# jasperlinthorst/reveal

Hardware: AMD Instinct MI355X
Metric: Mbp/s indexed+MUM-anchored (reveal rem) (higher is better)
Workload: dtype int32

## Files before the change

include/reveal_amd.h:

```cpp
#ifndef REVEAL_AMD_H
#define REVEAL_AMD_H
#include <stdint.h>

#ifdef __cplusplus
extern "C" {
#endif

typedef struct rv_index rv_index;

const char *rv_last_error(void);
int  rv_abi_version(void);
int  rv_sa_bits(void);
int  rv_device_count(void);

rv_index *rv_new(int device);
void rv_free(rv_index *h);

int rv_add_sample(rv_index *h);
int rv_add_sequence(rv_index *h, const char *seq, int64_t len, int64_t *begin, int64_t *end);
int rv_reset(rv_index *h);
int rv_reserve_text(rv_index *h, int64_t bytes);
int64_t rv_n(const rv_index *h);
int rv_nsamples(const rv_index *h);
int rv_nnodes(const rv_index *h);
// ... 12 lines not shown
int64_t rv_getmultimums(rv_index *h, int minlength, int minn, int mems, int64_t *members);
int rv_fetch_multi(rv_index *h, uint32_t *l, int32_t *n, int64_t *off, uint16_t *so, int64_t *pos);

typedef struct {
    int64_t n;
    int32_t depth;
    int32_t nsamples;
    int32_t nnodes;
    int32_t parent;
    int32_t kind;
    int32_t reserved;
    int64_t nmums;
    int64_t nmembers;
} rv_sub;

int rv_align_begin(rv_index *h, int minl, int minn);
int rv_frontier_size(rv_index *h);
int rv_frontier_scan(rv_index *h);
int rv_sub_skip_scan(rv_index *h, int s);
int rv_sub_info(rv_index *h, int s, rv_sub *out);
int rv_sub_nodes(rv_index *h, int s, int64_t *begin_end );
int rv_sub_mums(rv_index *h, int s, uint32_t *l, int32_t *n, int64_t *off, uint16_t *so, int64_t *pos);
int64_t rv_sub_array(rv_index *h, int s, int which, void *out, int64_t cap);
int rv_sub_split(rv_index *h, int s, uint32_t l, int nsp, const int64_t *sp,
                 const int64_t *lead, int nlead, const int64_t *trail, int ntrail,
                 const int64_t *match, int nmatch, const int64_t *rest, int nrest);
int rv_frontier_commit(rv_index *h, int32_t *children);
int rv_align_end(rv_index *h);

typedef struct {
    int64_t steps;
    int64_t splits;
    int64_t anchored_bp;
    int32_t levels;
    int32_t maxdepth;
    int64_t scanned_ranks;
    double  t_scan, t_host, t_split, t_bubble;
} rv_align_stats;
int rv_align_builtin(rv_index *h, int minl, int minn, rv_align_stats *st);

int rv_align_builtin_until(rv_index *h, int minl, int minn, int stop_subs, rv_align_stats *st);
int rv_align_builtin_resume(rv_index *h, rv_align_stats *st);
int rv_align_builtin_continue(rv_index *h, int stop_subs, rv_align_stats *st);
int rv_frontier_counts(rv_index *h, int64_t *out);
int rv_frontier_export(rv_index *h, int64_t *meta, int64_t *node_first, int64_t *nodes);
int64_t rv_frontier_pack(rv_index *h, const int32_t *subs, int k, void *sa, void *lcp, void *bwt, int on_device);
int rv_frontier_import(rv_index *h, int minl, int minn, uint32_t maxlcp, int level, int nsubs, const int64_t *meta,
                       const int64_t *node_first, const int64_t *nodes, int64_t m,
                       const void *sa, const void *lcp, const void *bwt, int on_device);
int64_t rv_frontier_seeds_export(rv_index *h, const int32_t *subs, int k, int64_t *out, int64_t cap);
int rv_frontier_seeds_import(rv_index *h, int nsubs, const int64_t *words, int64_t nwords);
uint32_t rv_maxlcp(const rv_index *h);
int rv_cascade_info(const rv_index *h, int64_t *out);
const char *rv_cascade_why(const rv_index *h);
int64_t rv_anchor_count(rv_index *h, int64_t *members);
int rv_fetch_anchors(rv_index *h, uint32_t *l, int64_t *off, int64_t *pos);
int rv_set_result_buffers(rv_index *h, uint32_t *l, int64_t l_cap, int64_t *off, int64_t off_cap, int64_t *pos, int64_t pos_cap);
typedef struct {
    int64_t  key, n;
    int32_t  depth, nsamples, nnodes, picked;
    int64_t  nmums;
    uint32_t l; int32_t mn;
    int64_t  sp_min;
    uint64_t h_sa, h_lcp, h_mums;
} rv_trace;
int rv_set_trace(rv_index *h, int on);
int rv_set_preselect(rv_index *h, int64_t maxmums);
int rv_set_option(rv_index *h, const char *name, int64_t value);
int rv_get_option(rv_index *h, const char *name, int64_t *value);
int rv_set_launch_trace(int on);
int rv_option_count(void);
const char *rv_option_name(int k);
int64_t rv_trace_count(rv_index *h);
int rv_fetch_trace(rv_index *h, rv_trace *out, int64_t cap);

typedef struct rv_subindex rv_subindex;
rv_index *rv_clone(rv_index *h);
rv_subindex *rv_sx_main(rv_index *h);
rv_subindex *rv_sx_copy(rv_subindex *x);
void rv_sx_free(rv_subindex *x);
int rv_sx_info(const rv_subindex *x, rv_sub *out);
int rv_sx_nodes(const rv_subindex *x, int64_t *begin_end);
int64_t rv_sx_array(rv_subindex *x, int which, void *out, int64_t cap);
int64_t rv_sx_scan(rv_subindex *x, int minl, int minn, int64_t *members);
int rv_sx_fetch(rv_subindex *x, uint32_t *l, int32_t *n, int64_t *off, uint16_t *so, int64_t *pos);
int rv_sx_split(rv_subindex *x, const int64_t *lead, int nlead, const int64_t *trail, int ntrail,
                const int64_t *match, int nmatch, const int64_t *rest, int nrest, rv_subindex **out);
int rv_sx_extract(rv_subindex *x, int64_t *intervals, int niv);

int64_t rv_chain(int64_t m, int k, const uint32_t *len, const int32_t *nmem, const int64_t *crd, const int64_t *left,
                 const int64_t *right, int64_t wscore, int64_t wpen, int model, int64_t *out_idx, int64_t *out_score);

typedef struct { int64_t wscore, wpen, maxmums, seedsize; int gcmodel; int trim; double pcutoff; } rv_picker_args;
typedef struct {
    int picked; uint32_t pick_l; int32_t pick_n; int pick_members; uint16_t *pick_so; int64_t *pick_pos; int64_t member_cap;
    int64_t nleft, nright, nseed_members, seed_cap, seed_member_cap;
    uint32_t *seed_l; int32_t *seed_n; int64_t *seed_off; uint16_t *seed_so; int64_t *seed_pos; int64_t *seed_score; uint8_t *seed_right;
} rv_picker_out;
int rv_set_picker(rv_index *h, int kind, const rv_picker_args *args);
int rv_picker_info(const rv_index *h, int64_t *out);
int rv_pick_chain(const rv_picker_args *args, int nsub, int64_t m, const uint32_t *l, const int32_t *n, const int64_t *off, const uint16_t *so,
                  const int64_t *pos, int nsamples, const int64_t *seq_begin, const int64_t *iv_begin, const int64_t *iv_end, int minlength,
                  rv_picker_out *out);

typedef struct rv_graph rv_graph;
rv_graph *rv_graph_import(int64_t nnodes, const int64_t *node_b, const int64_t *node_e, const int8_t *node_aligned, const int8_t *node_sent,
// ... 83 lines not shown
```

reveal_amd/_index.py:

```python
import ctypes
import mmap
import os
import sys
import numpy as np

from . import _lib
from ._lib import RV_T, RV_SA, RV_SAI, RV_LCP, RV_SO, RV_NSEP


def _page_array(count, dtype):
    nbytes = max(int(count), 1) * np.dtype(dtype).itemsize
    m = mmap.mmap(-1, (nbytes + mmap.PAGESIZE - 1) // mmap.PAGESIZE * mmap.PAGESIZE)
    return np.frombuffer(m, dtype=dtype, count=max(int(count), 1))


def _pairs(iv, sa64):
    a = np.ascontiguousarray(np.array([(int(b), int(e)) for b, e in iv], dtype=np.int64).reshape(-1, 2))
    return a, len(a)


_OPTION_DEFAULTS = {}


def make_index_type(sa64, error):
# ... 523 lines not shown
        def picker_info(self):
            o = (ctypes.c_int64 * 6)()
            self._dll.rv_picker_info(self._h, o)
            return dict(kind=int(o[0]), calls=int(o[1]), seeded=int(o[2]), picker_s=o[3] / 1e9, lists_s=o[4] / 1e9, graphalign_s=o[5] / 1e9)

        def _result_buffers_free(self):
            c = self.__dict__.get("_res_bufs")
            if c is not None and sys.getrefcount(c[0]) == 2 and sys.getrefcount(c[1]) == 2 and sys.getrefcount(c[2]) == 2:
                return c
            return None

        def _offer_result_buffers(self):
            c = self._result_buffers_free()
            if c is not None:
                self._dll.rv_set_result_buffers(self._h, c[0].ctypes.data, len(c[0]), c[1].ctypes.data, len(c[1]), c[2].ctypes.data, len(c[2]))
            else:
                self._dll.rv_set_result_buffers(self._h, None, 0, None, 0, None, 0)

        def _builtin_result(self, st, trace):
            dll, h = self._dll, self._h
            mem = ctypes.c_int64(0)
            na = dll.rv_anchor_count(h, ctypes.byref(mem))
            c = self._result_buffers_free()
            if c is not None and len(c[0]) >= max(na, 1) and len(c[1]) >= na + 1 and len(c[2]) >= max(mem.value, 1):
                l, off, pos = c
            else:
                dll.rv_set_result_buffers(h, None, 0, None, 0, None, 0)
                if os.environ.get("RV_RESULT_BUFS", "") == "heap":
                    l = np.empty(max(na, 1), dtype=np.uint32); off = np.empty(na + 1, dtype=np.int64); pos = np.empty(max(mem.value, 1), dtype=np.int64)
                else:
                    l = _page_array(max(na, 1), np.uint32); off = _page_array(na + 1, np.int64); pos = _page_array(max(mem.value, 1), np.int64)
                self.__dict__["_res_bufs"] = (l, off, pos)
            c = None
            off[0] = 0
            if dll.rv_fetch_anchors(h, l.ctypes.data, off.ctypes.data, pos.ctypes.data) != 0:
                self._fail()
            tr = None
            if trace:
                nt = dll.rv_trace_count(h)
                tr = np.zeros(max(nt, 1), dtype=_lib.TRACE_DTYPE)
                if dll.rv_fetch_trace(h, tr.ctypes.data, len(tr)) != 0:
                    self._fail()
                tr = tr[:nt]
            stats = {f[0]: getattr(st, f[0]) for f in _lib.RvAlignStats._fields_}
            return dict(stats=stats, anchors=(l[:na], off[:na + 1], pos[:mem.value]), trace=tr)

        @property
        def maxlcp(self):
            return int(self._dll.rv_maxlcp(self._h))

        def cascade_info(self):
            o = np.zeros(8, dtype=np.int64)
            self._dll.rv_cascade_info(self._h, o.ctypes.data)
            return dict(done=bool(o[0]), levels=int(o[1]), matches=int(o[2]), witnesses=int(o[3]), subindices=int(o[4]), undecided=int(o[5]), rebuilt_ranks=int(o[6]), decided_from_witnesses=int(o[7]),
                        why=(self._dll.rv_cascade_why(self._h) or b"").decode())

        def align_builtin_until(self, stop_subs, minl=20, minn=2, trace=False):
            if not self._constructed:
                raise error("Index not yet constructed, alignment stopped.")
            self._dll.rv_set_trace(self._h, 1 if trace else 0)
            self._offer_result_buffers()
            self._st = _lib.RvAlignStats()
            self._trace = bool(trace)
            r = self._dll.rv_align_builtin_until(self._h, int(minl), int(minn), int(stop_subs), ctypes.byref(self._st))
            if r < 0:
                self._fail()
            self._pending = r > 0
            return r

        def align_builtin_continue(self, stop_subs):
            if not getattr(self, "_pending", False):
                return 0
            self._offer_result_buffers()
            r = self._dll.rv_align_builtin_continue(self._h, int(stop_subs), ctypes.byref(self._st))
            if r < 0:
                self._fail()
            self._pending = r > 0
            return r

        def frontier(self):
            c = np.zeros(4, dtype=np.int64)
            if self._dll.rv_frontier_counts(self._h, c.ctypes.data) != 0:
                self._fail()
            ns, m, nn, level = (int(x) for x in c)
            meta = np.zeros((max(ns, 1), 6), dtype=np.int64); nf = np.zeros(ns + 1, dtype=np.int64); nodes = np.zeros((max(nn, 1), 2), dtype=np.int64)
            if self._dll.rv_frontier_export(self._h, meta.ctypes.data, nf.ctypes.data, nodes.ctypes.data) != 0:
                self._fail()
            return dict(level=level, m=m, meta=meta[:ns], node_first=nf, nodes=nodes[:nn])

        def frontier_pack(self, subs, sa, lcp, bwt):
            subs = np.ascontiguousarray(subs, dtype=np.int32)
            ptr, dev = _pointers(sa, lcp, bwt)
            r = self._dll.rv_frontier_pack(self._h, subs.ctypes.data, len(subs), ptr[0], ptr[1], ptr[2], dev)
            if r < 0:
                self._fail()
            return int(r)

        def frontier_seeds(self, subs):
            subs = np.ascontiguousarray(subs, dtype=np.int32)
            need = self._dll.rv_frontier_seeds_export(self._h, subs.ctypes.data, len(subs), None, 0)
            if need < 0:
                self._fail()
            out = np.zeros(max(int(need), 1), dtype=np.int64)
            if self._dll.rv_frontier_seeds_export(self._h, subs.ctypes.data, len(subs), out.ctypes.data, int(need)) != need:
                self._fail()
            return out[:int(need)]

# ... 69 lines not shown
```

reveal_amd/_lib.py:

```python
import ctypes
import importlib.util
import os
import sys
import numpy as np

_HERE = os.path.dirname(os.path.abspath(__file__))

RV_T, RV_SA, RV_SAI, RV_LCP, RV_SO, RV_NSEP, RV_NODES = range(7)
K_SCAN_PAIR, K_SCAN_MULTI, K_SA_SORT, K_LCP, K_SPLIT, K_LABEL, K_BUBBLE, K_RADIX_SCATTER, K_RADIX_HIST, K_TEXT_ROUND, K_CASCADE, K_DIAG_TABLE, K_INIT_KEYS, K_PUBLISH = range(14)

c_i64p = ctypes.POINTER(ctypes.c_int64)
V = ctypes.c_void_p


class RvSub(ctypes.Structure):
    _fields_ = [("n", ctypes.c_int64), ("depth", ctypes.c_int32), ("nsamples", ctypes.c_int32),
                ("nnodes", ctypes.c_int32), ("parent", ctypes.c_int32), ("kind", ctypes.c_int32),
                ("reserved", ctypes.c_int32), ("nmums", ctypes.c_int64), ("nmembers", ctypes.c_int64)]


class RvAlignStats(ctypes.Structure):
    _fields_ = [("steps", ctypes.c_int64), ("splits", ctypes.c_int64), ("anchored_bp", ctypes.c_int64),
                ("levels", ctypes.c_int32), ("maxdepth", ctypes.c_int32), ("scanned_ranks", ctypes.c_int64),
                ("t_scan", ctypes.c_double), ("t_host", ctypes.c_double), ("t_split", ctypes.c_double),
# ... 3 lines not shown
TRACE_DTYPE = np.dtype([("key", np.int64), ("n", np.int64), ("depth", np.int32), ("nsamples", np.int32),
                        ("nnodes", np.int32), ("picked", np.int32), ("nmums", np.int64), ("l", np.uint32),
                        ("mn", np.int32), ("sp_min", np.int64), ("h_sa", np.uint64), ("h_lcp", np.uint64),
                        ("h_mums", np.uint64)], align=True)

_I, _L, _D = ctypes.c_int, ctypes.c_int64, ctypes.c_double
SYMBOLS = {
    "rv_last_error": (ctypes.c_char_p, []),
    "rv_abi_version": (_I, []),
    "rv_sa_bits": (_I, []),
    "rv_device_count": (_I, []),
    "rv_new": (V, [_I]),
    "rv_free": (None, [V]),
    "rv_add_sample": (_I, [V]),
    "rv_add_sequence": (_I, [V, ctypes.c_char_p, _L, c_i64p, c_i64p]),
    "rv_reset": (_I, [V]),
    "rv_reserve_text": (_I, [V, _L]),
    "rv_n": (_L, [V]),
    "rv_nsamples": (_I, [V]),
    "rv_nnodes": (_I, [V]),
    "rv_node_list": (_I, [V, V]),
    "rv_construct": (_I, [V, _I, ctypes.c_char_p, ctypes.c_char_p, _I]),
    "rv_upload": (_I, [V]),
    "rv_upload_again": (_I, [V]),
    "rv_get_array": (_L, [V, _I, V, _L]),
    "rv_getmums": (_L, [V, _I]),
    "rv_fetch_mums": (_I, [V, V, V, V, _L]),
    "rv_getmultimums": (_L, [V, _I, _I, _I, c_i64p]),
    "rv_fetch_multi": (_I, [V, V, V, V, V, V]),
    "rv_align_begin": (_I, [V, _I, _I]),
    "rv_frontier_size": (_I, [V]),
    "rv_frontier_scan": (_I, [V]),
    "rv_sub_skip_scan": (_I, [V, _I]),
    "rv_sub_info": (_I, [V, _I, ctypes.POINTER(RvSub)]),
    "rv_sub_nodes": (_I, [V, _I, V]),
    "rv_sub_mums": (_I, [V, _I, V, V, V, V, V]),
    "rv_sub_array": (_L, [V, _I, _I, V, _L]),
    "rv_sub_split": (_I, [V, _I, ctypes.c_uint32, _I, V, V, _I, V, _I, V, _I, V, _I]),
    "rv_frontier_commit": (_I, [V, V]),
    "rv_align_end": (_I, [V]),
    "rv_align_builtin": (_I, [V, _I, _I, ctypes.POINTER(RvAlignStats)]),
    "rv_align_builtin_until": (_I, [V, _I, _I, _I, ctypes.POINTER(RvAlignStats)]),
    "rv_align_builtin_resume": (_I, [V, ctypes.POINTER(RvAlignStats)]),
    "rv_align_builtin_continue": (_I, [V, _I, ctypes.POINTER(RvAlignStats)]),
    "rv_frontier_counts": (_I, [V, V]),
    "rv_frontier_export": (_I, [V, V, V, V]),
    "rv_frontier_pack": (_L, [V, V, _I, V, V, V, _I]),
    "rv_frontier_import": (_I, [V, _I, _I, ctypes.c_uint32, _I, _I, V, V, V, _L, V, V, V, _I]),
    "rv_frontier_seeds_export": (_L, [V, V, _I, V, _L]),
    "rv_frontier_seeds_import": (_I, [V, _I, V, _L]),
    "rv_maxlcp": (ctypes.c_uint32, [V]),
    "rv_cascade_info": (ctypes.c_int, [V, V]),
    "rv_cascade_why": (ctypes.c_char_p, [V]),
    "rv_anchor_count": (_L, [V, c_i64p]),
    "rv_fetch_anchors": (_I, [V, V, V, V]),
    "rv_set_result_buffers": (_I, [V, V, _L, V, _L, V, _L]),
    "rv_set_trace": (_I, [V, _I]),
    "rv_set_preselect": (_I, [V, _L]),
    "rv_set_option": (_I, [V, ctypes.c_char_p, _L]),
    "rv_set_launch_trace": (_I, [_I]),
    "rv_batch_new": (V, []),
    "rv_batch_add": (_I, [V, V]),
    "rv_batch_run": (_I, [V, _I, _I, _I, V, V]),
    "rv_batch_info": (_I, [V, V]),
    "rv_batch_free": (None, [V]),
    "rv_dev_alloc": (V, [_I, _L]),
    "rv_dev_free": (_I, [_I, V]),
    "rv_ipc_export": (_I, [_I, V, V]),
    "rv_ipc_open": (V, [_I, V]),
    "rv_ipc_close": (_I, [_I, V]),
    "rv_dev_copy": (_I, [_I, V, V, _L]),
    "rv_get_option": (_I, [V, ctypes.c_char_p, c_i64p]),
    "rv_option_count": (_I, []),
    "rv_option_name": (ctypes.c_char_p, [_I]),
    "rv_trace_count": (_L, [V]),
    "rv_fetch_trace": (_I, [V, V, _L]),
    "rv_clone": (V, [V]),
    "rv_sx_main": (V, [V]),
    "rv_sx_copy": (V, [V]),
    "rv_sx_free": (None, [V]),
    "rv_sx_info": (_I, [V, ctypes.POINTER(RvSub)]),
    "rv_sx_nodes": (_I, [V, V]),
    "rv_sx_array": (_L, [V, _I, V, _L]),
    "rv_sx_scan": (_L, [V, _I, _I, c_i64p]),
    "rv_sx_fetch": (_I, [V, V, V, V, V, V]),
    "rv_sx_split": (_I, [V, V, _I, V, _I, V, _I, V, _I, V]),
    "rv_sx_extract": (_I, [V, V, _I]),
    "rv_chain": (_L, [_L, _I, V, V, V, V, V, _L, _L, _I, V, V]),
    "rv_prof_enable": (_I, [V, _I]),
    "rv_prof_reset": (_I, [V]),
    "rv_prof_get": (_I, [V, _I, c_i64p, ctypes.POINTER(_D), ctypes.POINTER(_D)]),
    "rv_measure_bandwidth": (_I, [_I, _L, _I, ctypes.POINTER(_D), ctypes.POINTER(_D)]),
    "rv_sa_stats": (_I, [V] + [ctypes.POINTER(_I)] * 4 + [c_i64p, ctypes.POINTER(_I)]),
    "rv_sa_diag_table": (_I, [V]),
    "rv_sa_tail": (_I, [V, c_i64p]),
    "rv_set_picker": (_I, [V, _I, V]),
    "rv_picker_info": (_I, [V, c_i64p]),
    "rv_pick_chain": (_I, [V, _I, _L, V, V, V, V, V, _I, V, V, V, _I, V]),
    "rv_graph_import": (V, [_L, V, V, V, V, V, V, V, _L, V, V, V, V, V, V, _I, V, V, _I, V, _I]),
    "rv_graph_pick": (_I, [V, V, _I, _L, V, V, V, V, V, V, V, _I, V]),
    "rv_graph_align": (_I, [V, V, _L, V, V, ctypes.c_uint32, V, _I, V, V]),
    "rv_graph_align_fetch": (_I, [V, V]),
    "rv_graph_finish": (_I, [V]),
    "rv_set_graph_picker": (_I, [V, V, V]),
    "rv_graph_new": (V, []),
    "rv_graph_replay_begin": (V, [_I, V, V]),
# ... 104 lines not shown
```

reveal_amd/csrc/rv_align.hip:

```cpp
#include "rv_index.h"
#include "rv_split.h"
#include "rv_decide.h"
static_assert(RV_TSUB_TILE == RV_SPLIT_TILE, "one tile -> sub-index table serves the split passes and the multi-sample picker");
#include "rv_leaf.h"
#include "rv_cascade.h"
#include <string.h>
#include <algorithm>
#include <chrono>
#include <thread>
#include <atomic>
#include "rv_graphrem.h"

namespace {

double now_s() {
    return std::chrono::duration<double>(std::chrono::steady_clock::now().time_since_epoch()).count();
}

u64 hash_step(u64 acc, u64 i, int64_t v) {
    u64 x = (u64)v + (i + 1) * 0x9E3779B97F4A7C15ULL;
    x ^= x >> 30; x *= 0xbf58476d1ce4e5b9ULL;
    x ^= x >> 27; x *= 0x94d049bb133111ebULL;
    x ^= x >> 31;
    return acc + x;
// ... 114 lines not shown
    DBuf dD, dTab, dTile, dList, dFlag, dPar, dDbg, scrSA, scrLCP, scrBWT;
    RvCascadeBufs cas;
    RvCascadeOut cas_out{};
    DBuf dPbReady; u32 pb_epoch = 0;
    DBuf dNextTsub;
    DBuf dTmin;
    HBuf hLeafRoots[2], hLeafOut;
    DBuf dLeaf, dLeafRoots[2];
    hipStream_t leaf_stream = nullptr, leaf_stream2 = nullptr;
    hipStream_t bub_stream = nullptr, bub_stream2 = nullptr;
    hipEvent_t ev_fork = nullptr, ev_join = nullptr, ev_join2 = nullptr;
    hipEvent_t ev_ready = nullptr, ev_leaf[RV_LEVEL_BUFS + 1] = {}, ev_roots[2] = {nullptr, nullptr};
    bool roots_inflight[2] = {false, false};
    bool flag_clean = false;
    DBuf dDec, dErr, dTab0;
    bool next_dev_ok = false, cur_dev_ok = false, early_done = false, early_bubble = false, use_leaf = false;
    int64_t par_min_cur = RV_BUBBLE_PAR_N;
    const sa_t *d_next_nodes = nullptr; const uint8_t *d_next_flags = nullptr;
    std::vector<sa_t> next_nodes; std::vector<uint8_t> next_flags;
    bool leaf_pending[RV_LEVEL_BUFS + 1] = {};
    size_t leaf_anchor_cap = 0, leaf_trace_cap = 0;
    std::vector<uint8_t> leaf_done;
    std::vector<RvLeafRoot> leaf_roots[2];
    Packer pk;
    std::vector<int> stamp; int epoch = 0;
    std::vector<sa_t> cb, ce, mb, me, cut_lo, cut_hi, mend_pos;
    std::vector<uint8_t> cc;
    std::vector<int> ctab_first, mtab_first, cut_first, mend_first, split_subs;
    std::vector<u32> sub_off_h;
    std::vector<int> tile_sub;
    std::vector<int64_t> mpre, sub_start, woff, toff, next_ss;
    const int64_t *d_next_ss = nullptr;
    const int *d_next_want = nullptr;
    const int *d_next_tsub = nullptr;
    std::vector<int> next_tsub;
    std::vector<u32> pick_l; std::vector<sa_t> pick_pos;
    std::vector<u32> child_base, child_n;
    std::vector<RvBubbleDesc> descs;
    std::vector<std::vector<RvBubbleDesc>> rounds;
    std::vector<RvBubbleDesc> kids_small, kids_big, kids_lds;
    struct Kid { int64_t off, n; int c0, c1; int64_t m0, wsum; };
    std::vector<Kid> kid_tmp;
    std::vector<u32> an_l; std::vector<int64_t> an_off, an_pos;
    bool trace_on = false;
    std::vector<rv_trace> trace;
    rv_align_stats st{};
    double lg[8] = {0}, lgx[8] = {0}, lg_t0 = 0;
    int leaf_flip = 0;
    bool leaf_launch_due = false, hook_early = false;
    size_t last_leaf_count = 0;
    bool running = false;
    u32 *lf_counters = nullptr; unsigned long long *lf_stats = nullptr; u32 *lf_l = nullptr; int64_t *lf_pos = nullptr; rv_trace *lf_tr = nullptr;
    size_t early_sent = 0; u32 *early_l = nullptr; int64_t *early_pos = nullptr;
    size_t leaf_na = 0;
    void release() {
        if (leaf_stream) (void)hipStreamSynchronize(leaf_stream);
        if (leaf_stream2) (void)hipStreamSynchronize(leaf_stream2);
        if (bub_stream) { (void)hipStreamSynchronize(bub_stream); (void)hipStreamSynchronize(bub_stream2); }
        for (int k = 0; k < RV_LEVEL_BUFS; k++) { lvSA[k].release(); lvLCP[k].release(); lvBWT[k].release(); }
        scrSA.release(); scrLCP.release(); scrBWT.release(); cas.release();
        dTmin.release(); dPbReady.release(); dNextTsub.release(); dD.release(); dTab.release(); dTile.release(); dList.release(); dFlag.release(); dPar.release(); dDbg.release(); pk.release(); dDec.release(); dErr.release(); dTab0.release(); hLeafRoots[0].release(); hLeafRoots[1].release(); hLeafOut.release(); dLeaf.release(); dLeafRoots[0].release(); dLeafRoots[1].release();
        if (leaf_stream) { rv_stream_put(leaf_stream); leaf_stream = nullptr; }
        if (leaf_stream2) { rv_stream_put(leaf_stream2); leaf_stream2 = nullptr; }
        if (bub_stream) { rv_stream_put(bub_stream); bub_stream = nullptr; rv_stream_put(bub_stream2); bub_stream2 = nullptr; (void)hipEventDestroy(ev_fork); (void)hipEventDestroy(ev_join); (void)hipEventDestroy(ev_join2); ev_fork = ev_join = ev_join2 = nullptr; }
        if (ev_ready) { (void)hipEventDestroy(ev_ready); ev_ready = nullptr; }
        for (int k = 0; k <= RV_LEVEL_BUFS; k++) if (ev_leaf[k]) { (void)hipEventDestroy(ev_leaf[k]); ev_leaf[k] = nullptr; }
        for (int k = 0; k < 2; k++) if (ev_roots[k]) { (void)hipEventDestroy(ev_roots[k]); ev_roots[k] = nullptr; }
    }
};

void rv_align_free(rv_index *h) {
    if (h->al && h->al->feed) { (void)rv_replay_feed_finish(h->al->feed); h->al->feed = nullptr; }
    if (h->al) { h->al->release(); delete h->al; h->al = nullptr; }
}

static int report_dev_err(u32 err) {
    if (err & 1u) { rv_set_error("split: the intervals returned by graphalign do not partition the sub-index (child size mismatch)"); return -1; }
    if (err & 4u) { rv_set_error("device-side decision: a picked match does not lie inside the intervals of its sub-index"); return -1; }
    if (err & 2u) { rv_set_error("bubble_sort (data-parallel rounds): a mover found no landing site"); return -1; }
    if (err & 16u) { rv_set_error("bubble_sort (data-parallel rounds): a tile waited in vain for the tile above it (workgroups not dispatched in index order?)"); return -1; }
    if (err) { rv_set_error("device-side error word %u", err); return -1; }
    return 0;
}

static int64_t bubble_par_default(bool multi) { return multi ? (int64_t)262144 : (int64_t)RV_BUBBLE_PAR_N; }

static const sa_t *cur_sa(rv_index *h) { Align *a = h->al; return a->level == 0 ? h->dSA.as<sa_t>() : a->lvSA[a->cur].as<sa_t>(); }
static const lcp_t *cur_lcp(rv_index *h) { Align *a = h->al; return a->level == 0 ? h->dLCP.as<lcp_t>() : a->lvLCP[a->cur].as<lcp_t>(); }
static const uint8_t *cur_bwt(rv_index *h) { Align *a = h->al; return a->level == 0 ? h->dBWT.as<uint8_t>() : a->lvBWT[a->cur].as<uint8_t>(); }

static int sample_of(const rv_index *h, int64_t pos) {
    return (int)(std::lower_bound(h->nsep.begin(), h->nsep.end(), pos) - h->nsep.begin());
}

static int count_samples(rv_index *h, const RvIntv *iv, size_t cnt) {
    Align *a = h->al;
    if (h->nsamples > 2) {
        bool sorted = true;
        for (size_t k = 1; k < cnt && sorted; k++) sorted = iv[k - 1].begin <= iv[k].begin;
        if (sorted) {
            int ns = 0, last = -1; size_t sp = 0;
            for (size_t k = 0; k < cnt; k++) {
                while (sp < h->nsep.size() && h->nsep[sp] < iv[k].begin) sp++;
                if ((int)sp != last) { ns++; last = (int)sp; }
            }
            return ns;
// ... 1119 lines not shown
    if (!a->multi && cm.m_next > 1) {
        a->d_err = a->dErr.as<u32>();
    } else {
        u32 err = 0;
        RV_HIP(hipMemcpyAsync(&err, a->dErr.p, 4, hipMemcpyDeviceToHost, q));
        RV_HIP(hipStreamSynchronize(q));
        RV_TRY(report_dev_err(err));
    }

    if (a->level == 0) h->main_arrays_freed = true;
    a->level++;
    a->cur = cm.nxt;
    a->cur_dev_ok = a->next_dev_ok; a->early_done = false; a->early_bubble = false;
    std::swap(a->lv, a->nx);
    a->dec.reset(a->lv.size());
    a->skip_scan.assign((size_t)a->lv.size(), 0);
    a->st.t_split += t1 - t0;
    a->st.t_bubble += now_s() - t1;
    return 0;
}

static int builtin_leaf_setup(rv_index *h) {
    Align *a = h->al;
    hipStream_t q = h->ws.stream;
    a->use_leaf = !a->multi && !h->ws.opt.no_leaf && a->picker == 0;
    a->leaf_flip = 0;
    if (!a->use_leaf) return 0;
    a->leaf_anchor_cap = (size_t)(h->nT / std::max(a->minl, 1)) + 1024;
    a->leaf_trace_cap = a->trace_on ? 2 * a->leaf_anchor_cap + 1024 : 0;
    const size_t bytes = 256 + a->leaf_anchor_cap * (4 + 8 + 8) + a->leaf_trace_cap * sizeof(rv_trace) + 64;
    RV_TRY(a->dLeaf.reserve(bytes));
    uint8_t *base = a->dLeaf.as<uint8_t>();
    a->lf_counters = (u32 *)base;
    a->lf_stats = (unsigned long long *)(base + 64);
    a->lf_pos = (int64_t *)(base + 256); a->lf_l = (u32 *)(a->lf_pos + 2 * a->leaf_anchor_cap);
    a->lf_tr = (rv_trace *)(base + 256 + a->leaf_anchor_cap * 20 + ((8 - (a->leaf_anchor_cap * 20) % 8) % 8));
    RV_HIP(hipMemsetAsync(base, 0, 256, q));
    if (!a->leaf_stream) {
        RV_HIP(rv_stream_get(&a->leaf_stream));
        RV_HIP(rv_stream_get(&a->leaf_stream2));
        RV_HIP(hipEventCreateWithFlags(&a->ev_ready, hipEventDisableTiming));
        for (int k = 0; k <= RV_LEVEL_BUFS; k++) RV_HIP(hipEventCreateWithFlags(&a->ev_leaf[k], hipEventDisableTiming));
        for (int k = 0; k < 2; k++) RV_HIP(hipEventCreateWithFlags(&a->ev_roots[k], hipEventDisableTiming));
    }
    for (int k = 0; k <= RV_LEVEL_BUFS; k++) a->leaf_pending[k] = false;
    a->roots_inflight[0] = a->roots_inflight[1] = false;
    return 0;
}

static int builtin_setup(rv_index *h, int minl, int minn) {
    RV_TRY(align_begin(h, minl, minn, h->al && h->al->trace_on));
    Align *a = h->al;
    a->full_only = !a->trace_on && a->picker == 0;
    a->an_l.clear(); a->an_off.assign(1, 0); a->an_pos.clear(); a->trace.clear(); a->leaf_na = 0; a->early_sent = 0;
    a->seeds_cur.clear(); a->seeds_lead.clear(); a->seeds_trail.clear(); a->picker_calls = a->picker_seeded = 0; a->picker_ns = a->picker_list_ns = a->galign_ns = 0;
    if (a->picker == 1) {
        if ((int)h->nodes.size() != h->nsamples) { rv_set_error("the native picker (rv_set_picker) takes one sequence per sample: %d sequences in %d samples", (int)h->nodes.size(), h->nsamples); return -1; }
        if (h->rc) { rv_set_error("the native picker (rv_set_picker) with construct(rc=1) is not supported"); return -1; }
    }
    if (a->picker != 0 && a->multi && !a->trace_on) { a->presel_on = true; a->pick_filter = true; }
    else a->pick_filter = false;
    if (a->picker == 2) {
        if (!a->ggraph) { rv_set_error("rv_set_graph_picker: no graph"); return -1; }
        if (h->rc) { rv_set_error("the native picker (rv_set_graph_picker) with construct(rc=1) is not supported"); return -1; }
        a->g_left.assign((size_t)a->lv.size(), RvGraphIv{-1, -1}); a->g_right.assign((size_t)a->lv.size(), RvGraphIv{-1, -1});
    }
    const bool use_leaf = !a->multi && !h->ws.opt.no_leaf && a->picker == 0;
    a->use_leaf = use_leaf;
    if (!a->multi && a->full_only && h->n < ((int64_t)1 << 32)) {
        prep_level_tables(h, a->lv, h->n);
        if (a->next_dev_ok) {
            a->pk.clear();
            RV_TRY(publish_next_tables(h, a->dTab0, a->lv.nsamples, false));
            a->cur_dev_ok = true;
        }
    }
    RV_TRY(builtin_leaf_setup(h));
    a->running = true;
    return 0;
}

struct PickScratch {
    std::vector<u32> pk_l, pk_sl; std::vector<int32_t> pk_n, pk_sn; std::vector<int64_t> pk_off, pk_mpos, pk_sb, pk_ib, pk_ie, pk_soff, pk_spos, pk_ssc;
    std::vector<uint16_t> pk_mso, pk_sso; std::vector<uint8_t> pk_srt;
};
struct PickRes {
    int rc = -9;
    u32 l = 0; int members = 0;
    std::vector<uint16_t> so; std::vector<int64_t> pos;
    double t_list = 0, t_pick = 0;
    std::string err;
};
static void pick_one(rv_index *h, int s, PickScratch &X, PickRes &R, RvGraphIv gleft = RvGraphIv{-1, -1}, RvGraphIv gright = RvGraphIv{-1, -1}) {
    Align *a = h->al;
    const Level &lv = a->lv;
    const int W = h->nsamples, want = lv.nsamples[(size_t)s];
    const RvIntv *nodes = lv.nodes.data() + lv.node_first[(size_t)s];
    const size_t nn = (size_t)(lv.node_first[(size_t)s + 1] - lv.node_first[(size_t)s]);
    const int64_t first = a->mum_first[(size_t)s], cnt = a->nmums[(size_t)s];
    Align::SeedList &sl = a->seeds_lead[(size_t)s], &st = a->seeds_trail[(size_t)s];
    R.so.assign((size_t)W, 0); R.pos.assign((size_t)W, 0);
    const double tp0 = now_s();
    X.pk_l.clear(); X.pk_n.clear(); X.pk_off.assign(1, 0); X.pk_mso.clear(); X.pk_mpos.clear();
    if (!a->multi) {
        for (int64_t k = first; k < first + cnt; k++) {
            const RvPairRec &r = a->recs[(size_t)k];
            X.pk_l.push_back(r.l); X.pk_n.push_back(2);
// ... 312 lines not shown
            fprintf(stderr, "level %3d subs %7d (leaf %7zu) ranks %10lld | leafprep %6.1f scan %6.1f host %6.1f | commit: tables %6.1f upload %6.1f split-enq %6.1f bubble-enq %6.1f | drain %7.1f us | next biggest %lld\n",
                    log_level, log_ns, log_leaf, (long long)log_m, (tl_leaf - tl0) * 1e6, (t0 - tl_leaf) * 1e6, (tl1 - t0) * 1e6,
                    a->lg[0] * 1e6, (a->lg[1] - a->lg[0]) * 1e6, (a->lg[2] - a->lg[1]) * 1e6, (tl2 - tl1) * 1e6 - a->lg[2] * 1e6, (tl3 - tl2) * 1e6,
                    (long long)biggest);
        }
    }
    RV_HIP(hipStreamSynchronize(q));
    if (a->lv.size() > 0) {
        u32 err = 0;
        RV_HIP(hipMemcpy(&err, a->dErr.p, 4, hipMemcpyDeviceToHost));
        if (err & 1u) { rv_set_error("split: the intervals returned by graphalign do not partition the sub-index (child size mismatch)"); return -1; }
        if (err) { rv_set_error("device-side error %u in the level before the hand-off", err); return -1; }
    }
    return 0;
}

static void fill_offsets(int64_t *off, size_t na, int64_t base) {
    const int nt = na > ((size_t)1 << 18) ? 4 : 1;
    std::vector<std::thread> th;
    for (int t = 1; t < nt; t++) {
        const size_t lo = na / nt * t, hi = t + 1 == nt ? na : na / nt * (t + 1);
        th.emplace_back([=]() { for (size_t k = lo; k < hi; k++) off[k] = base + 2 * (int64_t)(k + 1); });
    }
    for (size_t k = 0; k < na / nt; k++) off[k] = base + 2 * (int64_t)(k + 1);
    for (auto &x : th) x.join();
}
static int builtin_finish(rv_index *h, rv_align_stats *out) {
    Align *a = h->al;
    hipStream_t q = h->ws.stream;
    h->rb.direct = false;
    if (a->use_leaf && a->running) {
        u32 *lf_counters = a->lf_counters; u32 *lf_l = a->lf_l; int64_t *lf_pos = a->lf_pos; rv_trace *lf_tr = a->lf_tr;
        RV_HIP(hipStreamSynchronize(a->leaf_stream));
        RV_HIP(hipStreamSynchronize(a->leaf_stream2));
        for (int k = 0; k <= RV_LEVEL_BUFS; k++) a->leaf_pending[k] = false;
        RV_TRY(a->hLeafOut.reserve(256));
        RV_HIP(hipMemcpyAsync(a->hLeafOut.p, lf_counters, 128, hipMemcpyDeviceToHost, q));
        RV_HIP(hipStreamSynchronize(q));
        u32 cnt[4]; unsigned long long stv[8];
        memcpy(cnt, a->hLeafOut.p, sizeof cnt); memcpy(stv, a->hLeafOut.as<uint8_t>() + 64, sizeof stv);
        if (h->ws.opt.leaf_prof)
            fprintf(stderr, "leaf: steps %llu splits %llu | cycles idle %llu scan %llu split %llu bubble %llu\n", stv[0], stv[1], stv[4], stv[5], stv[6], stv[7]);
        if (cnt[2]) { rv_set_error(cnt[2] & 4u ? "leaf kernel: recursion stack overflow" : "leaf kernel: a sub-index does not match its intervals"); return -1; }
        if (cnt[0] > a->leaf_anchor_cap || cnt[1] > a->leaf_trace_cap) { rv_set_error("leaf kernel: output buffer too small"); return -1; }
        a->leaf_na = 0;
        if (cnt[0]) {
            const size_t na = cnt[0];
            const size_t nl = a->an_l.size(), np = a->an_pos.size();
            rv_index::ResultBufs &rb = h->rb;
            rb.direct = rb.l && (int64_t)(nl + na) <= rb.l_cap && (int64_t)(nl + na + 1) <= rb.off_cap && (int64_t)(np + 2 * na) <= rb.pos_cap;
            int64_t *pp; u32 *pl;
            if (rb.direct) { pp = rb.pos + np; pl = rb.l + nl; }
            else { RV_TRY(a->hLeafOut.reserve(na * 20 + 64)); pp = a->hLeafOut.as<int64_t>(); pl = (u32 *)(pp + 2 * na); }
            const size_t sent = (rb.direct && a->early_l == pl && a->early_pos == pp) ? std::min(a->early_sent, na) : 0;
            if (sent < na) {
                RV_HIP(hipMemcpyAsync(pp + 2 * sent, lf_pos + 2 * sent, (na - sent) * 16, hipMemcpyDeviceToHost, a->leaf_stream));
                RV_HIP(hipMemcpyAsync(pl + sent, lf_l + sent, (na - sent) * 4, hipMemcpyDeviceToHost, a->leaf_stream));
            }
            RV_TRY(rv_ensure_working_text(h));
            RV_TRY(rv_leaf_lower_launch(h->ws, h->dT.as<uint8_t>(), lf_pos, lf_l, (u32)na));
            if (rb.direct) fill_offsets(rb.off + nl + 1, na, (int64_t)np);
            RV_HIP(hipStreamSynchronize(a->leaf_stream));
            RV_HIP(hipStreamSynchronize(q));
            a->leaf_na = na;
        }
        if (a->trace_on && cnt[1]) {
            const size_t at = a->trace.size();
            a->trace.resize(at + cnt[1]);
            RV_HIP(hipMemcpy(a->trace.data() + at, lf_tr, (size_t)cnt[1] * sizeof(rv_trace), hipMemcpyDeviceToHost));
        }
        a->st.steps += (int64_t)stv[0]; a->st.splits += (int64_t)stv[1]; a->st.anchored_bp += (int64_t)stv[2];
        if ((int64_t)stv[3] > a->st.maxdepth) a->st.maxdepth = (int32_t)stv[3];
    }
    a->running = false;
    if (out) *out = a->st;
    return 0;
}

static int install_frontier(rv_index *h, int level, int nsubs, const int64_t *meta, const int64_t *node_first, const int64_t *nodes, int64_t m,
                            const void *sa, const void *lcp, const void *bwt, int on_device);
static int builtin_cascade(rv_index *h) {
    Align *a = h->al;
    memset(&a->cas_out, 0, sizeof a->cas_out);
    if (a->trace_on || h->rc != 0 || h->n <= RV_LEAF_N || a->minl < 4 || h->ws.opt.no_cascade || a->picker != 0) return 0;
    const bool second_try = !a->multi && a->use_leaf && h->ws.opt.cascade_second == 2;
    auto interval_cascade = [&]() -> int {
        RvCascadeMultiOut mo;
        RV_TRY(rv_cascade_multi_run(h, a->cas, a->minl, &mo));
        a->cas_out.done = mo.done; a->cas_out.levels = mo.levels; a->cas_out.cands = mo.cands; a->cas_out.witnesses = mo.witnesses; a->cas_out.children = mo.children;
        a->cas_out.undecided = mo.undecided; a->cas_out.rebuilt_ranks = mo.rebuilt_ranks; a->cas_out.why = mo.why;
        if (!mo.done) return 0;
        const int k = h->nsamples;
        a->st.splits += (int64_t)mo.an_l.size(); a->st.steps += mo.steps; a->st.levels += mo.levels; a->st.scanned_ranks += h->n;
        if (mo.maxdepth > a->st.maxdepth) a->st.maxdepth = mo.maxdepth;
        h->main_arrays_freed = true;
        if (mo.undecided > 0) {
            RV_TRY(install_frontier(h, 1, (int)mo.undecided, mo.meta.data(), mo.node_first.data(), mo.nodes.data(), mo.rebuilt_ranks, mo.d_sa, mo.d_lcp, mo.d_bwt, 1));
        } else {
            a->lv.clear();
            a->level = 1;
        }
        {
            const size_t na = mo.an_l.size(), l0 = a->an_l.size(), p0 = a->an_pos.size(), o0 = a->an_off.size();
            a->an_l.insert(a->an_l.end(), mo.an_l.begin(), mo.an_l.end());
            a->an_pos.resize(p0 + na * (size_t)k);
            for (size_t x = 0; x < na * (size_t)k; x++) a->an_pos[p0 + x] = (int64_t)mo.an_pos[x];
            a->an_off.resize(o0 + na);
            for (size_t x = 0; x < na; x++) a->an_off[o0 + x] = (int64_t)(p0 + (x + 1) * (size_t)k);
            int64_t bp = 0;
            for (size_t x = 0; x < na; x++) bp += mo.an_l[x];
            a->st.anchored_bp += bp;
            (void)l0;
        }
        return 0;
    };
    if (a->multi || second_try) return interval_cascade();
    if (!a->use_leaf) return 0;
    RvCascadeIO io;
    io.anchor_count = a->lf_counters; io.anchor_cap = (u32)a->leaf_anchor_cap; io.anchor_l = a->lf_l; io.anchor_pos = a->lf_pos;
    io.stats = a->lf_stats; io.leaf_err = a->lf_counters + 2;
    io.stage_cap = (u32)h->ws.opt.leaf_acap;
    RvCascadeHost hx;
    hx.side = a->leaf_stream;
    a->early_sent = 0;
    if (h->rb.l) {
        const int64_t nl = (int64_t)a->an_l.size(), np = (int64_t)a->an_pos.size();
        const int64_t room = std::min(std::min(h->rb.l_cap - nl, h->rb.off_cap - nl - 1), (h->rb.pos_cap - np) / 2);
        if (room > 0) { hx.l = h->rb.l + nl; hx.pos = h->rb.pos + np; hx.cap = (u32)std::min<int64_t>(room, 0xffffffffll); }
    }
    io.lvSA = &a->lvSA[0]; io.lvLCP = &a->lvLCP[0]; io.lvBWT = &a->lvBWT[0]; io.roots = &a->dLeafRoots[0];
    const int dmode = (int)h->ws.opt.cascade_danger;
    RV_TRY(rv_cascade_run(h, a->cas, io, a->minl, &a->cas_out, dmode == 2 ? 1 : 0, 0, &hx));
    if (!a->cas_out.done && a->cas_out.undecided > 0 && dmode == 1) {
        RV_HIP(hipMemsetAsync(a->dLeaf.p, 0, 256, h->ws.stream));
        RV_TRY(rv_cascade_run(h, a->cas, io, a->minl, &a->cas_out, 1, 1, &hx));
    }
    if (!a->cas_out.done) {
        if (hx.l) RV_HIP(hipStreamSynchronize(a->leaf_stream));
        RV_HIP(hipMemsetAsync(a->dLeaf.p, 0, 256, h->ws.stream));
        if (a->cas_out.undecided > 0 && !h->ws.opt.cascade_second_off) return interval_cascade();
        return 0;
    }
    a->st.levels += a->cas_out.levels;
    a->st.scanned_ranks += h->n;
    a->early_sent = a->cas_out.sent; a->early_l = hx.l; a->early_pos = hx.pos;
    if (!a->cas.lin_rest.empty() && h->nodes.size() > 2) {
        std::vector<RvIntv> rest, gone;
        for (size_t k = 0; k + 1 < a->cas.lin_rest.size(); k += 2) rest.push_back({a->cas.lin_rest[k], a->cas.lin_rest[k + 1]});
        std::sort(rest.begin(), rest.end(), intv_less);
        for (const RvIntv &v : h->nodes) {
            if (v.end <= v.begin) continue;
            const auto it = std::lower_bound(rest.begin(), rest.end(), v, intv_less);
            if (it == rest.end() || it->begin != v.begin) gone.push_back(v);
        }
        RV_TRY(add_decision(h, 0, 0, nullptr, 0, gone.data(), (int)gone.size(), nullptr, 0, nullptr, 0, rest.data(), (int)rest.size()));
        a->dec.drop_lead = true;
        RV_TRY(rv_frontier_commit(h, nullptr));
        for (size_t s2 = 0; s2 < a->lv.depth.size(); s2++) a->lv.depth[s2] = a->cas.lin_rest_depth;
        return 0;
    }
    h->main_arrays_freed = true;
    a->level = 1;
    a->lv.clear();
    return 0;
}

int rv_cascade_info(const rv_index *h, int64_t *out) {
    for (int k = 0; k < 8; k++) out[k] = 0;
    if (!h->al) return 0;
    const RvCascadeOut &c = h->al->cas_out;
    out[0] = c.done ? 1 : 0; out[1] = c.levels; out[2] = c.cands; out[3] = c.witnesses; out[4] = c.children; out[5] = c.undecided; out[6] = c.rebuilt_ranks; out[7] = c.solved;
    return 0;
}

const char *rv_cascade_why(const rv_index *h) {
    if (!h->al || h->al->cas_out.done || !h->al->cas_out.why) return "";
    return h->al->cas_out.why;
}

int rv_align_builtin(rv_index *h, int minl, int minn, rv_align_stats *out) {
    RV_TRY(builtin_setup(h, minl, minn));
    Align *a = h->al;
    if (a->replay_graph && a->picker == 1) {
        a->feed = rv_replay_feed_start(a->replay_graph);
        a->fed = 0;
        a->replay_graph = nullptr;
        if (!a->feed) return -1;
    }
    int rc = builtin_cascade(h);
    if (rc == 0) rc = builtin_levels(h, 0);
    if (rc == 0) rc = builtin_finish(h, out);
    if (a->feed) {
        RvReplayFeed *f = a->feed; a->feed = nullptr;
        if (rc == 0) { if (rv_replay_feed_finish(f) != 0) return -1; }
        else { const std::string keep = rv_last_error(); (void)rv_replay_feed_finish(f); rv_set_error("%s", keep.c_str()); }
    }
    return rc;
}

int rv_align_builtin_until(rv_index *h, int minl, int minn, int stop_subs, rv_align_stats *out) {
    RV_TRY(builtin_setup(h, minl, minn));
    RV_TRY(builtin_cascade(h));
    RV_TRY(builtin_levels(h, stop_subs));
    Align *a = h->al;
    if (a->lv.size() == 0) { RV_TRY(builtin_finish(h, out)); return 0; }
    if (out) *out = a->st;
    return a->lv.size();
}

int rv_align_builtin_continue(rv_index *h, int stop_subs, rv_align_stats *out) {
    RV_TRY(need_align(h));
    if (!h->al->running) { rv_set_error("no built-in run in progress (rv_align_builtin_until / rv_frontier_import)"); return -1; }
    if (stop_subs < 1) { rv_set_error("rv_align_builtin_continue: stop_subs must be positive"); return -1; }
    RV_HIP(hipSetDevice(h->device));
    Align *a = h->al;
    RV_TRY(builtin_levels(h, std::max(stop_subs, a->lv.size() + 1)));
    if (a->lv.size() == 0) { RV_TRY(builtin_finish(h, out)); return 0; }
    if (out) *out = a->st;
    return a->lv.size();
}

int rv_align_builtin_resume(rv_index *h, rv_align_stats *out) {
    RV_TRY(need_align(h));
    if (!h->al->running) { rv_set_error("no built-in run in progress (rv_align_builtin_until / rv_frontier_import)"); return -1; }
// ... 77 lines not shown
    a->level = std::max(level, 1);
    a->cur = 0;
    RV_TRY(a->lvSA[0].reserve((size_t)(m + 64) * sizeof(sa_t)));
    RV_TRY(a->lvLCP[0].reserve((size_t)(m + 64) * sizeof(lcp_t)));
    RV_TRY(a->lvBWT[0].reserve((size_t)m + 64));
    const hipMemcpyKind kind = on_device ? hipMemcpyDeviceToDevice : hipMemcpyHostToDevice;
    if (m) {
        RV_HIP(hipMemcpyAsync(a->lvSA[0].p, sa, (size_t)m * sizeof(sa_t), kind, q));
        RV_HIP(hipMemcpyAsync(a->lvLCP[0].p, lcp, (size_t)m * sizeof(lcp_t), kind, q));
        RV_HIP(hipMemcpyAsync(a->lvBWT[0].p, bwt, (size_t)m, kind, q));
    }
    prep_level_tables(h, lv, m);
    a->pk.clear();
    RV_TRY(publish_next_tables(h, a->dTab0, lv.nsamples, false));
    RV_HIP(hipStreamSynchronize(q));
    a->cur_dev_ok = a->next_dev_ok; a->early_done = false; a->early_bubble = false;
    a->scanned = false; a->d_err = nullptr;
    a->dec.reset(lv.size());
    a->skip_scan.assign((size_t)lv.size(), 0);
    a->seeds_cur.clear(); a->seeds_lead.clear(); a->seeds_trail.clear();
    return 0;
}


int rv_frontier_import(rv_index *h, int minl, int minn, uint32_t maxlcp, int level, int nsubs, const int64_t *meta,
                       const int64_t *node_first, const int64_t *nodes, int64_t m, const void *sa, const void *lcp, const void *bwt, int on_device) {
    RV_HIP(hipSetDevice(h->device));
    if (h->nsamples < 2) { rv_set_error("align needs at least two samples"); return -1; }
    if (nsubs < 0 || m < 0 || m >= ((int64_t)1 << 32)) { rv_set_error("rv_frontier_import: bad sizes"); return -1; }
    const bool fresh = !(h->al && h->al->running);
    if (fresh) {
        if (h->text_only) h->maxlcp = maxlcp;
        else if (!h->constructed || h->main_arrays_freed) RV_TRY(rv_text_only(h, maxlcp));
        const bool keep_trace = h->al && h->al->trace_on;
        if (!h->al) h->al = new Align();
        Align *a = h->al;
        a->trace_on = keep_trace;
        a->minl = minl; a->minn = minn;
        a->multi = h->nsamples > 2;
        a->scanned = false; a->d_err = nullptr; a->flag_clean = false;
        a->next_dev_ok = a->cur_dev_ok = a->early_done = a->early_bubble = false;
        a->par_min_cur = (h->ws.opt.bubble_par_min >= 0 ? h->ws.opt.bubble_par_min : bubble_par_default(a->multi));
        RV_TRY(a->dErr.reserve(64));
        memset(&a->st, 0, sizeof a->st);
        a->full_only = !a->trace_on && a->picker == 0;
        a->pick_filter = a->picker != 0 && a->multi && !a->trace_on;
        if (a->pick_filter) a->presel_on = true;
        if (a->picker == 2) { rv_set_error("rv_frontier_import: a run on a graph (rv_set_graph_picker) is not handed off -- its sub-indices share the graph"); return -1; }
        if (a->picker == 1) {
            if ((int)h->nodes.size() != h->nsamples) { rv_set_error("the native picker (rv_set_picker) takes one sequence per sample: %d sequences in %d samples", (int)h->nodes.size(), h->nsamples); return -1; }
            if (h->rc) { rv_set_error("the native picker (rv_set_picker) with construct(rc=1) is not supported"); return -1; }
        }
        a->picker_calls = a->picker_seeded = 0; a->picker_ns = a->picker_list_ns = a->galign_ns = 0;
        a->an_l.clear(); a->an_off.assign(1, 0); a->an_pos.clear(); a->trace.clear(); a->leaf_na = 0; a->early_sent = 0;
        RV_TRY(builtin_leaf_setup(h));
    }
    RV_TRY(install_frontier(h, level, nsubs, meta, node_first, nodes, m, sa, lcp, bwt, on_device));
    h->al->running = true;
    return 0;
}

int64_t rv_frontier_seeds_export(rv_index *h, const int32_t *subs, int k, int64_t *out, int64_t cap) {
    if (need_align(h)) return -1;
    const Align *a = h->al;
    const int ns = a->lv.size();
    int64_t need = 0;
    for (int pass = 0; pass < 2; pass++) {
        int64_t at = 0;
        for (int i = 0; i < k; i++) {
            const int s = subs[i];
            if (s < 0 || s >= ns) { rv_set_error("sub-index %d out of range", s); return -1; }
            const Align::SeedList *sd = (s < (int)a->seeds_cur.size() && a->seeds_cur[(size_t)s].size() > 0) ? &a->seeds_cur[(size_t)s] : nullptr;
            if (pass) out[at] = sd ? (int64_t)sd->size() : 0;
            at++;
            if (!sd) continue;
            for (size_t r = 0; r < sd->size(); r++) {
                const int64_t mem = sd->off[r + 1] - sd->off[r];
                if (pass) {
                    out[at] = sd->l[r]; out[at + 1] = sd->n[r]; out[at + 2] = sd->score[r]; out[at + 3] = mem;
                    for (int64_t q2 = 0; q2 < mem; q2++) { out[at + 4 + 2 * q2] = sd->so[(size_t)(sd->off[r] + q2)]; out[at + 5 + 2 * q2] = sd->pos[(size_t)(sd->off[r] + q2)]; }
                }
                at += 4 + 2 * mem;
            }
        }
        need = at;
        if (!out || cap < need) break;
    }
    return need;
}

int rv_frontier_seeds_import(rv_index *h, int nsubs, const int64_t *words, int64_t nwords) {
    RV_TRY(need_align(h));
    Align *a = h->al;
    if (!a->running || nsubs != a->lv.size()) { rv_set_error("rv_frontier_seeds_import: %d seed lists for a frontier of %d sub-indices", nsubs, a->lv.size()); return -1; }
    if (a->picker != 1) { rv_set_error("rv_frontier_seeds_import: seeds belong to the native picker (rv_set_picker)"); return -1; }
    std::vector<Align::SeedList> nxt((size_t)nsubs);
    int64_t at = 0;
    for (int s = 0; s < nsubs; s++) {
        if (at >= nwords) { rv_set_error("rv_frontier_seeds_import: truncated seed lists"); return -1; }
        const int64_t cnt = words[at++];
        if (cnt < 0) { rv_set_error("rv_frontier_seeds_import: bad seed count"); return -1; }
        for (int64_t r = 0; r < cnt; r++) {
            if (at + 4 > nwords) { rv_set_error("rv_frontier_seeds_import: truncated seed lists"); return -1; }
            const int64_t l = words[at], n = words[at + 1], sc = words[at + 2], mem = words[at + 3];
            if (mem < 0 || mem > h->nsamples || at + 4 + 2 * mem > nwords) { rv_set_error("rv_frontier_seeds_import: bad seed record"); return -1; }
            std::vector<uint16_t> so((size_t)mem); std::vector<int64_t> pos((size_t)mem);
            for (int64_t q2 = 0; q2 < mem; q2++) {
// ... 350 lines not shown
```

reveal_amd/csrc/rv_cascade.h:

```cpp
#pragma once
#include "rv_common.h"
#include <vector>

struct RvCascadeBufs {
    DBuf d[40];
    HBuf hstage, hstage2;
    u32 M = 0, NW = 0;
    u32 lin_roots = 0, lin_picks = 0, lin_nA = 0, lin_nB = 0;
    int64_t lin_steps = 0; int lin_maxdepth = 0; size_t lin_off[6] = {0, 0, 0, 0, 0, 0};
    std::vector<int64_t> lin_rest; int lin_rest_depth = 0;
    hipStream_t prio_stream = nullptr; hipEvent_t ev_in = nullptr, ev_out = nullptr;
    void release() {
        for (auto &b : d) b.release(); hstage.release(); hstage2.release();
        if (prio_stream) { (void)hipStreamDestroy(prio_stream); prio_stream = nullptr; }
        if (ev_in) { (void)hipEventDestroy(ev_in); ev_in = nullptr; }
        if (ev_out) { (void)hipEventDestroy(ev_out); ev_out = nullptr; }
    }
};

struct RvCascadeIO {
    u32 *anchor_count; u32 anchor_cap; u32 *anchor_l; int64_t *anchor_pos;
    unsigned long long *stats;
    u32 *leaf_err;
    u32 stage_cap;
    DBuf *lvSA, *lvLCP, *lvBWT, *roots;
};

struct RvCascadeHost {
    hipStream_t side = nullptr;
    int64_t *pos = nullptr; u32 *l = nullptr; u32 cap = 0;
};

struct RvCascadeOut {
    bool done;
    int levels;
    int64_t cands, witnesses, children, undecided, rebuilt_ranks;
    int64_t solved, unsolved;
    const char *why;
    u32 sent;
};

#define RV_CASM_K 16
struct RvCascadeMultiOut {
    bool done; int levels; int64_t cands, witnesses, children, undecided, rebuilt_ranks, steps; int maxdepth; const char *why;
    int64_t big, big_ranks;
    std::vector<u32> an_l; std::vector<int64_t> an_pos;
    std::vector<int64_t> meta, node_first, nodes;
    const void *d_sa, *d_lcp, *d_bwt;
};

struct rv_index;
struct RvBatchGroup;
RvBatchGroup *rv_batch_group_new(int device);
void rv_batch_group_begin(RvBatchGroup *g, int total);
void rv_batch_group_leave(RvBatchGroup *g);
void rv_batch_group_free(RvBatchGroup *g);
void rv_batch_group_info(const RvBatchGroup *g, int64_t *out);
int rv_cascade_multi_run(rv_index *h, RvCascadeBufs &cb, int minl, RvCascadeMultiOut *out);
int rv_cascade_run(rv_index *h, RvCascadeBufs &cb, const RvCascadeIO &io, int minl, RvCascadeOut *out, int danger = 0, int reuse = 0,
                   const RvCascadeHost *host = nullptr);
```

reveal_amd/csrc/rv_cascade.hip:

```cpp
#include "rv_index.h"
#include "rv_cascade.h"
#include "rv_leaf.h"
#include <algorithm>
#include <string.h>
#include <stdio.h>
#include <stdlib.h>
#include <chrono>

namespace {

constexpr int TB = 256;
constexpr u32 NONE = 0xFFFFFFFFu;
#ifdef RV_SA64
constexpr int KEY_SHIFT = 40;
#else
constexpr int KEY_SHIFT = 32;
#endif
constexpr u64 KEY_LOW = (1ull << KEY_SHIFT) - 1;

struct CasIv { sa_t a0, a1, b0, b1; };
struct CasRes { sa_t qa, qb; u32 ql, lead, trail, state; };
enum { C_NCHILD = 0, C_NUND = 1, C_NWIT = 2, C_ERR = 3, C_MAXN = 4, C_LO = 5, C_HI = 6, C_LEVELS = 7, C_NSOLVED = 8, C_NUNSOLVED = 9, C_NRETRY = 10, C_TICKET = 11,
       C_NANCH = 12  };

__device__ inline bool cas_cut(const CasIv &iv, int64_t pa, int64_t pb, int64_t len, int64_t minl, int64_t *qa, int64_t *qb, int64_t *ql) {
    const int64_t ka = (int64_t)iv.a0 - pa, kb = (int64_t)iv.b0 - pb;
    int64_t k = ka > kb ? ka : kb;
    k = k > 0 ? k : 0;
    const int64_t a = pa + k, b = pb + k;
    int64_t l = len - k;
    const int64_t ra = (int64_t)iv.a1 - a, rb = (int64_t)iv.b1 - b;
    l = l < ra ? l : ra;
    l = l < rb ? l : rb;
    *qa = a; *qb = b; *ql = l;
    return l >= minl;
}
__device__ inline u64 cas_key(int64_t qa, int64_t ql) { return ((u64)ql << KEY_SHIFT) | (KEY_LOW - (u64)qa); }

__device__ inline u64 shfl_up64(u64 v, int d) {
    const u32 lo = __shfl_up((u32)v, d, 64), hi = __shfl_up((u32)(v >> 32), d, 64);
    return ((u64)hi << 32) | lo;
}
__device__ inline void seg_atomic_max64(u64 *__restrict__ dst, u32 child, u64 val, bool active) {
    const int lane = threadIdx.x & 63;
    if (!active) { child = NONE; val = 0; }
    val = rv_wave_seg_max_u64(child, val);
    const u32 nc = __shfl_down(child, 1, 64);
    const bool last = lane == 63 || nc != child;
    if (active && last && val > dst[child]) atomicMax((unsigned long long *)&dst[child], (unsigned long long)val);
}
__device__ inline void seg_atomic_max32(u32 *__restrict__ dst, u32 child, u32 val, bool active) {
    const int lane = threadIdx.x & 63;
    if (!active) { child = NONE; val = 0; }
    val = rv_wave_seg_max_u32(child, val);
    const u32 nc = __shfl_down(child, 1, 64);
    const bool last = lane == 63 || nc != child;
    if (active && last && val > dst[child]) atomicMax(&dst[child], val);
}

constexpr int WT_ITEMS = 8;
constexpr int WT_TILE = TB * WT_ITEMS;
constexpr int WT_REGIONS = 64;
__global__ __launch_bounds__(TB) void k_cas_witness(const sa_t *__restrict__ SA, const lcp_t *__restrict__ LCP, const uint8_t *__restrict__ BWT, int64_t n,
                                                    u32 minl, sa_t *__restrict__ w_pos, u32 *__restrict__ w_val, u32 *__restrict__ w_rank, u32 cap , u32 *__restrict__ counters ) {
    __shared__ __attribute__((aligned(16))) u32 sl0[WT_TILE + 8];
    __shared__ __attribute__((aligned(16))) uint8_t ss0[WT_TILE + 32];
    u32 *const sl = sl0 + 3;
    uint8_t *const ss = ss0 + 15;
    const int64_t j0 = (int64_t)blockIdx.x * WT_TILE;
    if (j0 + WT_TILE + 2 <= n && sizeof(lcp_t) == 4) {
        const uint4 *L4 = reinterpret_cast<const uint4 *>(LCP + j0);
        uint4 *d4 = reinterpret_cast<uint4 *>(sl + 1);
        for (int k = threadIdx.x; k < WT_TILE / 4; k += TB) d4[k] = L4[k];
        const uint4 *B4 = reinterpret_cast<const uint4 *>(BWT + j0);
        for (int k = threadIdx.x; k < WT_TILE / 16; k += TB) {
            uint4 v = B4[k];
            v.x = (v.x >> 7) & 0x01010101u; v.y = (v.y >> 7) & 0x01010101u; v.z = (v.z >> 7) & 0x01010101u; v.w = (v.w >> 7) & 0x01010101u;
            reinterpret_cast<uint4 *>(ss + 1)[k] = v;
        }
        if (threadIdx.x == 0) { sl[0] = j0 > 0 ? (u32)LCP[j0 - 1] : 0u; ss[0] = j0 > 0 ? (uint8_t)(BWT[j0 - 1] >> 7) : (uint8_t)0; }
        if (threadIdx.x == 1) { sl[WT_TILE + 1] = (u32)LCP[j0 + WT_TILE]; ss[WT_TILE + 1] = (uint8_t)(BWT[j0 + WT_TILE] >> 7); }
        if (threadIdx.x == 2) sl[WT_TILE + 2] = (u32)LCP[j0 + WT_TILE + 1];
    } else {
        for (int k = threadIdx.x; k < WT_TILE + 3; k += TB) { const int64_t j = j0 - 1 + k; sl[k] = (j >= 0 && j < n) ? (u32)LCP[j] : 0u; }
        for (int k = threadIdx.x; k < WT_TILE + 2; k += TB) { const int64_t j = j0 - 1 + k; ss[k] = (j >= 0 && j < n) ? (uint8_t)(BWT[j] >> 7) : (uint8_t)0; }
    }
    __syncthreads();
    const int lane = threadIdx.x & 63;
    const u64 lt = (lane == 0) ? 0ull : (~0ull >> (64 - lane));
#pragma unroll 1
    for (int r = 0; r < WT_ITEMS; r++) {
        const int k = r * TB + threadIdx.x;
        const int64_t j = j0 + k;
        const u32 lm1 = sl[k], l0 = sl[k + 1], l1 = sl[k + 2], l2 = sl[k + 3];
        const u32 sm1 = ss[k], s0 = ss[k + 1], s1 = ss[k + 2];
        const bool pair0 = (j >= 1) & (l0 > lm1) & (l0 > l1) & (s0 != sm1);
        const bool pair1 = (j + 1 < n) & (l1 > l0) & (l1 > l2) & (s1 != s0);
        const u32 w = pair0 ? (lm1 > l1 ? lm1 : l1) : pair1 ? (l0 > l2 ? l0 : l2) : (l0 > l1 ? l0 : l1);
        const bool hit = (j < n) & (w >= minl);
        const u64 bal = __ballot(hit);
        if (bal) {
            const u32 reg = blockIdx.x & (WT_REGIONS - 1);
            u32 base = 0;
            if (lane == 0) base = atomicAdd(&counters[reg], (u32)__popcll(bal));
            base = (u32)__shfl((int)base, 0, 64);
            if (hit) {
                const u32 i = base + (u32)__popcll(bal & lt);
                if (i < cap) { w_pos[(size_t)reg * cap + i] = SA[j]; w_val[(size_t)reg * cap + i] = w; w_rank[(size_t)reg * cap + i] = (u32)j; }
            }
        }
    }
}
__global__ __launch_bounds__(TB) void k_cas_wpack(const sa_t *__restrict__ src_pos, const u32 *__restrict__ src_val, const u32 *__restrict__ src_rank, u32 rcap,
                                                  const u32 *__restrict__ region_cnt, const u32 *__restrict__ region_off, sa_t *__restrict__ w_pos, u32 *__restrict__ w_val,
                                                  u32 *__restrict__ w_rank) {
    const u32 reg = blockIdx.y, i = blockIdx.x * TB + threadIdx.x;
    if (i >= region_cnt[reg]) return;
    const size_t f = (size_t)reg * rcap + i;
    const u32 o = region_off[reg] + i;
    w_pos[o] = src_pos[f]; w_val[o] = src_val[f]; w_rank[o] = src_rank[f];
}
__global__ __launch_bounds__(TB) void k_cas_wkeys(const u32 *__restrict__ w_rank, u32 NW, u64 *__restrict__ keys, u32 *__restrict__ vals) {
    const u32 i = blockIdx.x * TB + threadIdx.x;
    if (i < NW) { keys[i] = (u64)w_rank[i]; vals[i] = i; }
}
__global__ __launch_bounds__(TB) void k_cas_wgather(const sa_t *__restrict__ src_pos, const u32 *__restrict__ src_val, const u32 *__restrict__ perm, u32 NW,
                                                    sa_t *__restrict__ w_pos, u32 *__restrict__ w_val) {
    const u32 i = blockIdx.x * TB + threadIdx.x;
    if (i < NW) { const u32 f = perm[i]; w_pos[i] = src_pos[f]; w_val[i] = src_val[f]; }
}

__global__ __launch_bounds__(TB) void k_cas_keys(const RvPairRec *__restrict__ recs, u32 M, u64 *__restrict__ keys, u32 *__restrict__ vals) {
    const u32 i = blockIdx.x * TB + threadIdx.x;
    if (i < M) { keys[i] = (u64)recs[i].a; vals[i] = i; }
}
__global__ __launch_bounds__(TB) void k_cas_gather(const RvPairRec *__restrict__ recs, const u32 *__restrict__ perm, u32 M, sa_t *__restrict__ c_pa,
                                                   sa_t *__restrict__ c_pb, u32 *__restrict__ c_len, u32 *__restrict__ c_child) {
    const u32 i = blockIdx.x * TB + threadIdx.x;
    if (i >= M) return;
    const RvPairRec r = recs[perm[i]];
    c_pa[i] = r.a; c_pb[i] = r.b; c_len[i] = r.l; c_child[i] = 0u;
}
__global__ void k_cas_init(CasIv *__restrict__ iv, u64 *__restrict__ best, u32 *__restrict__ wmax, int32_t *__restrict__ depth, CasRes *__restrict__ res,
                           u32 *__restrict__ counters, CasIv root, u32 *__restrict__ w_child, u32 nw, u64 *__restrict__ dbest, u32 *__restrict__ dflag, u64 *__restrict__ dceil) {
    const u32 i = blockIdx.x * blockDim.x + threadIdx.x;
    if (i == 0) {
        if (dbest) { dbest[0] = 0; dflag[0] = 0; dceil[0] = 0; }
        iv[0] = root; best[0] = 0; wmax[0] = 0; depth[0] = 0;
        CasRes r; r.qa = 0; r.qb = 0; r.ql = 0; r.lead = NONE; r.trail = NONE; r.state = 0;
        res[0] = r;
        counters[C_NCHILD] = 1; counters[C_NUND] = 0; counters[C_ERR] = 0; counters[C_MAXN] = 0; counters[C_LO] = 0; counters[C_HI] = 1; counters[C_LEVELS] = 0; counters[C_NSOLVED] = 0; counters[C_NUNSOLVED] = 0; counters[C_NRETRY] = 0; counters[C_TICKET] = 0;
    }
    if (i < nw) w_child[i] = 0u;
}

struct CasRootTabs { const sa_t *beginA, *beginB; const int32_t *pickA, *pickB; const u32 *rootLead, *rootTrail; u32 nA, nB; };
__device__ inline int cas_contig_of(const sa_t *__restrict__ begins, u32 cnt, int64_t pos) {
    u32 lo = 0, hi = cnt;
    while (lo < hi) { const u32 mid = (lo + hi) >> 1; if ((int64_t)begins[mid] <= pos) lo = mid + 1; else hi = mid; }
    return (int)lo - 1;
}
__global__ void k_cas_init_roots(CasIv *__restrict__ iv, u64 *__restrict__ best, u32 *__restrict__ wmax, int32_t *__restrict__ depth, CasRes *__restrict__ res,
                                 u32 *__restrict__ counters, const CasIv *__restrict__ roots, const int32_t *__restrict__ rdepth, u32 nroots,
                                 u64 *__restrict__ dbest, u32 *__restrict__ dflag, u64 *__restrict__ dceil) {
    const u32 i = blockIdx.x * blockDim.x + threadIdx.x;
    if (i == 0) {
        counters[C_NCHILD] = nroots; counters[C_NUND] = 0; counters[C_ERR] = 0; counters[C_MAXN] = 0; counters[C_LO] = 0; counters[C_HI] = nroots; counters[C_LEVELS] = 0;
        counters[C_NSOLVED] = 0; counters[C_NUNSOLVED] = 0; counters[C_NRETRY] = 0; counters[C_TICKET] = 0;
    }
    if (i < nroots) {
        if (dbest) { dbest[i] = 0; dflag[i] = 0; dceil[i] = 0; }
        iv[i] = roots[i]; best[i] = 0; wmax[i] = 0; depth[i] = rdepth[i];
// ... 2 lines not shown
    }
}
__global__ __launch_bounds__(TB) void k_cas_assign_roots(const sa_t *__restrict__ c_pa, const sa_t *__restrict__ c_pb, const u32 *__restrict__ c_len, u32 *__restrict__ c_child, u32 M,
                                                         const sa_t *__restrict__ w_pos, u32 *__restrict__ w_child, u32 NW, const CasIv *__restrict__ roots, CasRootTabs t, int64_t minl) {
    const u32 i = blockIdx.x * TB + threadIdx.x;
    if (i < M) {
        const int64_t pa = (int64_t)c_pa[i], pb = (int64_t)c_pb[i], len = (int64_t)c_len[i];
        const int ca = cas_contig_of(t.beginA, t.nA, pa), cb = cas_contig_of(t.beginB, t.nB, pb);
        u32 c = NONE;
        if (ca >= 0 && cb >= 0 && t.pickA[ca] >= 0 && t.pickA[ca] == t.pickB[cb]) {
            const u32 k = (u32)t.pickA[ca];
            int64_t qa, qb, ql;
            if (t.rootLead[k] != NONE && cas_cut(roots[t.rootLead[k]], pa, pb, len, minl, &qa, &qb, &ql)) c = t.rootLead[k];
            else if (t.rootTrail[k] != NONE && cas_cut(roots[t.rootTrail[k]], pa, pb, len, minl, &qa, &qb, &ql)) c = t.rootTrail[k];
        }
        c_child[i] = c;
    }
    if (i < NW) {
        const int64_t pos = (int64_t)w_pos[i];
        const bool a_side = t.nB == 0 || pos < (int64_t)t.beginB[0];
        const int ct = a_side ? cas_contig_of(t.beginA, t.nA, pos) : cas_contig_of(t.beginB, t.nB, pos);
        u32 c = NONE;
        if (ct >= 0) {
            const int32_t k = a_side ? t.pickA[ct] : t.pickB[ct];
            if (k >= 0) {
                for (int which = 0; which < 2 && c == NONE; which++) {
                    const u32 r = which ? t.rootTrail[k] : t.rootLead[k];
                    if (r == NONE) continue;
                    const CasIv p = roots[r];
                    if ((pos >= (int64_t)p.a0 && pos < (int64_t)p.a1) || (pos >= (int64_t)p.b0 && pos < (int64_t)p.b1)) c = r;
                }
            }
        }
        w_child[i] = c;
    }
}
__global__ void k_cas_lineage_stats(unsigned long long *__restrict__ stats, unsigned long long steps, unsigned long long maxdepth) {
    if (threadIdx.x == 0 && blockIdx.x == 0) { atomicAdd(&stats[0], steps); atomicMax(&stats[3], maxdepth); }
}
__global__ __launch_bounds__(TB) void k_cas_lkeys(const sa_t *__restrict__ c_pa, const u32 *__restrict__ c_len, u32 M, u64 *__restrict__ keys, u32 *__restrict__ vals) {
    const u32 i = blockIdx.x * TB + threadIdx.x;
    if (i < M) { keys[i] = (((1ull << (64 - KEY_SHIFT)) - 1ull - (u64)c_len[i]) << KEY_SHIFT) | (u64)c_pa[i]; vals[i] = i; }
}
__global__ __launch_bounds__(TB) void k_cas_lgather(const sa_t *__restrict__ c_pa, const sa_t *__restrict__ c_pb, const u32 *__restrict__ c_len, const u32 *__restrict__ perm, u32 M,
                                                    sa_t *__restrict__ o_pa, sa_t *__restrict__ o_pb, u32 *__restrict__ o_len) {
    const u32 i = blockIdx.x * TB + threadIdx.x;
    if (i < M) { const u32 f = perm[i]; o_pa[i] = c_pa[f]; o_pb[i] = c_pb[f]; o_len[i] = c_len[f]; }
}

constexpr int CAS_ITEMS = 4;
__global__ __launch_bounds__(TB) void k_cas_assign(const sa_t *__restrict__ c_pa, const sa_t *__restrict__ c_pb, const u32 *__restrict__ c_len, u32 *__restrict__ c_child,
                                                   u32 M, const sa_t *__restrict__ w_pos, const u32 *__restrict__ w_val, u32 *__restrict__ w_child, u32 NW,
                                                   const CasIv *__restrict__ iv, const CasRes *__restrict__ res, u64 *__restrict__ best, u32 *__restrict__ wmax,
                                                   int64_t minl, int first, const u64 *__restrict__ ceil ) {
    const u32 mblocks = (M + TB * CAS_ITEMS - 1) / (TB * CAS_ITEMS);
    for (int it = 0; it < CAS_ITEMS; it++) {
    if (blockIdx.x < mblocks) {
        const u32 i = (blockIdx.x * CAS_ITEMS + (u32)it) * TB + threadIdx.x;
        u32 c = i < M ? c_child[i] : NONE;
        bool live = c != NONE;
        u64 key = 0;
        if (live) {
            const int64_t pa = (int64_t)c_pa[i], pb = (int64_t)c_pb[i], len = (int64_t)c_len[i];
            int64_t qa, qb, ql;
            if (!first) {
                const CasRes r = res[c];
                const CasIv p = iv[c];
                u32 nc = NONE;
                if (r.state == 1u) {
                    CasIv lv; lv.a0 = p.a0; lv.a1 = r.qa; lv.b0 = p.b0; lv.b1 = r.qb;
                    CasIv tv; tv.a0 = (sa_t)((int64_t)r.qa + r.ql); tv.a1 = p.a1; tv.b0 = (sa_t)((int64_t)r.qb + r.ql); tv.b1 = p.b1;
                    if (r.lead != NONE && cas_cut(lv, pa, pb, len, minl, &qa, &qb, &ql)) nc = r.lead;
                    else if (r.trail != NONE && cas_cut(tv, pa, pb, len, minl, &qa, &qb, &ql)) nc = r.trail;
                } else if (r.state == 3u) {
                    if (cas_cut(p, pa, pb, len, minl, &qa, &qb, &ql)) nc = r.lead;
                }
                c = nc;
                c_child[i] = c;
                live = c != NONE;
            } else {
                live = cas_cut(iv[c], pa, pb, len, minl, &qa, &qb, &ql);
                if (!live) { c = NONE; c_child[i] = NONE; }
            }
            if (live) key = cas_key(qa, ql);
        }
        bool bid = live;
        if (live && ceil) { const u64 ce = ceil[c]; bid = ce == 0 || key < ce; }
        seg_atomic_max64(best, c, key, bid);
    } else {
        const u32 i = ((blockIdx.x - mblocks) * CAS_ITEMS + (u32)it) * TB + threadIdx.x;
        u32 c = i < NW ? w_child[i] : NONE;
        bool live = c != NONE;
        u32 v = 0;
        if (live) {
            const int64_t pos = (int64_t)w_pos[i];
            v = w_val[i];
            if (!first) {
                const CasRes r = res[c];
                const CasIv p = iv[c];
                u32 nc = NONE;
                if (r.state == 1u) {
                    const int64_t ea = (int64_t)r.qa + r.ql, eb = (int64_t)r.qb + r.ql;
                    const bool in_lead = (pos >= p.a0 && pos < r.qa) || (pos >= p.b0 && pos < r.qb);
                    const bool in_trail = (pos >= ea && pos < p.a1) || (pos >= eb && pos < p.b1);
                    nc = in_lead ? r.lead : in_trail ? r.trail : NONE;
                } else if (r.state == 3u) nc = r.lead;
                c = nc;
                w_child[i] = c;
                live = c != NONE;
            } else {
                const CasIv p = iv[c];
                live = (pos >= p.a0 && pos < p.a1) || (pos >= p.b0 && pos < p.b1);
                if (!live) { c = NONE; w_child[i] = NONE; }
            }
        }
        seg_atomic_max32(wmax, c, v, live);
    }
    }
}

__global__ __launch_bounds__(TB) void k_cas_winner(const sa_t *__restrict__ c_pa, const sa_t *__restrict__ c_pb, const u32 *__restrict__ c_len,
                                                   const u32 *__restrict__ c_child, u32 M, const CasIv *__restrict__ iv, CasRes *__restrict__ res,
                                                   const u64 *__restrict__ best, int64_t minl) {
    const u32 i = blockIdx.x * TB + threadIdx.x;
    if (i >= M) return;
    const u32 c = c_child[i];
    if (c == NONE) return;
    int64_t qa, qb, ql;
    if (!cas_cut(iv[c], (int64_t)c_pa[i], (int64_t)c_pb[i], (int64_t)c_len[i], minl, &qa, &qb, &ql)) return;
    if (cas_key(qa, ql) == best[c]) { res[c].qa = (sa_t)qa; res[c].qb = (sa_t)qb; res[c].ql = (u32)ql; }
}

constexpr u32 DWALK = 1024;
struct CasDanger { u64 *best; u32 *flag; sa_t *qb; u64 *ceil; u32 *m1, *p1, *m2; u64 *key; const uint8_t *T0; const lcp_t *LCP; const u64 *rank; u32 leaf_n; uint8_t *dflag; const uint8_t *wcls; };
__device__ inline bool cas_is_danger(const CasIv &p, u64 bk, u32 wm, u32 minl, u32 leaf_n, u32 *theta) {
    const int64_t la = (int64_t)p.a1 - p.a0, lb = (int64_t)p.b1 - p.b0;
    const u32 bl = (u32)(bk >> KEY_SHIFT);
    const bool can = (la >= (int64_t)minl) & (lb >= (int64_t)minl);
    const bool split = can & (bl >= minl) & (bl > wm);
    *theta = bl >= minl ? bl : minl;
    return can & !split & (wm >= minl) & ((u64)(la + lb) > (u64)leaf_n);
}
__global__ __launch_bounds__(TB) void k_cas_dmark(const CasIv *__restrict__ iv, const u64 *__restrict__ best, const u32 *__restrict__ wmax, u32 minl, const u32 *__restrict__ counters, CasDanger dg) {
    const u32 lo = counters[C_LO], hi = counters[C_HI];
    for (u32 id = lo + blockIdx.x * TB + threadIdx.x; id < hi; id += gridDim.x * TB) {
        u32 theta;
        dg.dflag[id] = cas_is_danger(iv[id], best[id], wmax[id], minl, dg.leaf_n, &theta) ? 1 : 0;
    }
}
__global__ __launch_bounds__(TB) void k_cas_dwalk(const sa_t *__restrict__ w_pos, const u32 *__restrict__ w_val, const u32 *__restrict__ w_child, u32 NW,
                                                  const CasIv *__restrict__ iv, const u64 *__restrict__ best, const u32 *__restrict__ wmax, u32 minl, CasDanger dg) {
    const u32 i = blockIdx.x * TB + threadIdx.x;
    if (i >= NW) return;
    if (dg.wcls && dg.wcls[i]) return;
    const u32 c = w_child[i];
    if (c == NONE || !dg.dflag[c]) return;
    dg.m1[i] = 0; dg.key[i] = 0;
    const CasIv p = iv[c];
    u32 theta;
    if (!cas_is_danger(p, best[c], wmax[c], minl, dg.leaf_n, &theta)) return;
    const int64_t pos = (int64_t)w_pos[i];
    const int64_t cap = (pos < (int64_t)p.a1 ? (int64_t)p.a1 : (int64_t)p.b1) - pos;
    if (w_val[i] < theta || cap < (int64_t)theta) return;
    u32 b1 = 0, b2 = 0, part = NONE;
    bool over = false;
#pragma unroll 1
    for (int dir = -1; dir <= 1; dir += 2) {
        u32 steps = 0;
        u64 rk = dg.rank[i];
        u32 run = 0xFFFFFFFFu;
        for (int64_t k = (int64_t)i + dir; k >= 0 && k < (int64_t)NW; k += dir) {
            const u64 r2 = dg.rank[k];
            if (r2 != rk + (u64)(int64_t)dir) break;
            const u32 g = (u32)dg.LCP[dir > 0 ? r2 : rk];
            run = g < run ? g : run;
            rk = r2;
            if (run < theta) break;
            if (++steps > DWALK) { over = true; break; }
// ... 85 lines not shown
                u32 l = (u32)(cap < ck ? cap : ck);
                l = run < l ? run : l;
                if (l > b1) { b2 = b1; b1 = l; part = s0 + (u32)k; }
                else if (l > b2) b2 = l;
                if (run <= b2) break;
            }
        }
        dg.m1[i] = b1 >= theta ? b1 : 0u; dg.p1[i] = part; dg.m2[i] = b2;
    }
}
__global__ __launch_bounds__(TB) void k_cas_dpick(const sa_t *__restrict__ w_pos, const u32 *__restrict__ w_val, const u32 *__restrict__ w_child, u32 NW,
                                                  const CasIv *__restrict__ iv, const CasRes *__restrict__ res, const u64 *__restrict__ best, const u32 *__restrict__ wmax,
                                                  u32 minl, CasDanger dg) {
    const u32 i = blockIdx.x * TB + threadIdx.x;
    if (i >= NW) return;
    const u32 c = w_child[i];
    if (c == NONE || !dg.dflag[c]) return;
    const CasIv p = iv[c];
    u32 theta;
    const u64 bk = best[c];
    if (!cas_is_danger(p, bk, wmax[c], minl, dg.leaf_n, &theta)) return;
    const int64_t pos = (int64_t)w_pos[i];
    const int64_t cap = (pos < (int64_t)p.a1 ? (int64_t)p.a1 : (int64_t)p.b1) - pos;
    if (w_val[i] < theta || cap < (int64_t)theta) return;
    if ((u32)(bk >> KEY_SHIFT) >= minl) { const CasRes r = res[c]; if (pos == (int64_t)r.qa || pos == (int64_t)r.qb) atomicOr(&dg.flag[c], 1u); }
    const u32 b1 = dg.m1[i];
    if (b1 == 0) return;
    const u32 w = dg.p1[i];
    if (dg.m1[w] != b1 || dg.p1[w] != i || b1 <= dg.m2[i] || b1 <= dg.m2[w]) return;
    const int64_t pw = (int64_t)w_pos[w];
    const bool a_side = pos < (int64_t)p.a1, w_a_side = pw < (int64_t)p.a1;
    if (!a_side || w_a_side) return;
    const int64_t qa = pos, qb = pw;
    if (!(qa == (int64_t)p.a0 || qb == (int64_t)p.b0)) {
        const uint8_t ca = dg.T0[qa - 1];
        if (ca == dg.T0[qb - 1] && ca != 'N' && ca != '$' && !(ca >= 'a' && ca <= 'z')) return;
    }
    const u64 key = cas_key(qa, (int64_t)b1);
    dg.key[i] = key;
    if (key > dg.best[c]) atomicMax((unsigned long long *)&dg.best[c], (unsigned long long)key);
}
__global__ __launch_bounds__(TB) void k_cas_dwrite(const sa_t *__restrict__ w_pos, const u32 *__restrict__ w_child, u32 NW, CasDanger dg) {
    const u32 i = blockIdx.x * TB + threadIdx.x;
    if (i >= NW) return;
    const u32 c = w_child[i];
    if (c == NONE || !dg.dflag[c]) return;
    const u64 key = dg.key[i];
    if (key == 0) return;
    if (key == dg.best[c]) dg.qb[c] = w_pos[dg.p1[i]];
}

__global__ __launch_bounds__(TB) void k_cas_decide(CasIv *__restrict__ iv, u64 *__restrict__ best, u32 *__restrict__ wmax, int32_t *__restrict__ depth,
                                                   CasRes *__restrict__ res, u32 minl, u32 *__restrict__ counters, u32 child_cap,
                                                   u32 *__restrict__ und_list, u32 leaf_n, RvCascadeIO io, CasDanger dg, int danger) {
    __shared__ u32 s_cnt[TB / 64][3];
    __shared__ u32 s_base[3];
    const u32 lo = counters[C_LO], hi = counters[C_HI];
    const int lane = threadIdx.x & 63, w = threadIdx.x >> 6;
    const u64 lt = (lane == 0) ? 0ull : (~0ull >> (64 - lane));
    for (u32 first = lo + blockIdx.x * TB; first < hi; first += gridDim.x * TB) {
        const u32 id = first + threadIdx.x;
        const bool in = id < hi;
        CasIv p; p.a0 = p.a1 = p.b0 = p.b1 = 0;
        u64 bk = 0; u32 wm = 0; int32_t dp = 0;
        CasRes r; r.qa = r.qb = 0; r.ql = 0; r.lead = r.trail = NONE; r.state = 2;
        if (in) { p = iv[id]; bk = best[id]; wm = wmax[id]; dp = depth[id]; r = res[id]; }
        const int64_t la = (int64_t)p.a1 - p.a0, lb = (int64_t)p.b1 - p.b0;
        const u32 bl = (u32)(bk >> KEY_SHIFT);
        const bool can = in & (la >= (int64_t)minl) & (lb >= (int64_t)minl);
        bool split = can & (bl >= minl) & (bl > wm);
        bool und = can & !split & (wm >= minl);
        bool forced = false, retry = false;
        if (danger && und && (u64)(la + lb) > (u64)dg.leaf_n) {
            const u32 fl = dg.flag[id];
            const u64 kh = dg.best[id], kc = (bl >= minl && !(fl & 1u)) ? bk : 0ull;
            if (!(fl & 2u)) {
                if (kh == 0 && kc == 0) {
                    if (bl < minl) und = false;
                    else if ((fl >> 8) < 16u) { retry = true; und = false; }
                } else {
                    if (kh > kc) { r.qa = (sa_t)(KEY_LOW - (kh & KEY_LOW)); r.qb = dg.qb[id]; r.ql = (u32)(kh >> KEY_SHIFT); }
                    split = true; forced = true; und = false;
                }
            }
            if (!retry) atomicAdd(&counters[und ? C_NUNSOLVED : C_NSOLVED], 1u);
        }
        bool lead = retry, trail = false;
        if (split) {
            if (!forced && r.ql != bl) atomicOr(&counters[C_ERR], 2u);
            lead = ((int64_t)r.qa - p.a0) + ((int64_t)r.qb - p.b0) > 0;
            trail = ((int64_t)p.a1 - r.qa - r.ql) + ((int64_t)p.b1 - r.qb - r.ql) > 0;
        }
        const u64 b_lead = __ballot(lead), b_trail = __ballot(trail), b_split = __ballot(split), b_und = __ballot(und);
        if (retry) atomicAdd(&counters[C_NRETRY], 1u);
        if (lane == 0) { s_cnt[w][0] = (u32)__popcll(b_lead) + (u32)__popcll(b_trail); s_cnt[w][1] = (u32)__popcll(b_split); s_cnt[w][2] = (u32)__popcll(b_und); }
        __syncthreads();
        if (threadIdx.x < 3) {
            u32 tot = 0;
            for (int k = 0; k < TB / 64; k++) tot += s_cnt[k][threadIdx.x];
            u32 *ctr = threadIdx.x == 0 ? &counters[C_NCHILD] : threadIdx.x == 1 ? io.anchor_count : &counters[C_NUND];
            s_base[threadIdx.x] = tot ? atomicAdd(ctr, tot) : 0u;
        }
        __syncthreads();
        u32 base_c = s_base[0], base_a = s_base[1], base_u = s_base[2];
        for (int k = 0; k < w; k++) { base_c += s_cnt[k][0]; base_a += s_cnt[k][1]; base_u += s_cnt[k][2]; }
        if (retry) {
            const u32 slot = base_c + (u32)__popcll(b_lead & lt) + (u32)__popcll(b_trail & lt);
            CasRes nr; nr.qa = 0; nr.qb = 0; nr.ql = 0; nr.lead = NONE; nr.trail = NONE; nr.state = 0;
            if (slot < child_cap) {
                iv[slot] = p; best[slot] = 0; wmax[slot] = 0; depth[slot] = dp; res[slot] = nr;
                dg.best[slot] = 0; dg.flag[slot] = ((dg.flag[id] >> 8) + 1u) << 8; dg.ceil[slot] = bk;
                r.lead = slot; r.trail = NONE;
            } else atomicOr(&counters[C_ERR], 1u);
            r.state = 3;
        } else if (split) {
            u32 slot = base_c + (u32)__popcll(b_lead & lt) + (u32)__popcll(b_trail & lt);
            CasRes nr; nr.qa = 0; nr.qb = 0; nr.ql = 0; nr.lead = NONE; nr.trail = NONE; nr.state = 0;
            if (lead) {
                if (slot < child_cap) {
                    CasIv c; c.a0 = p.a0; c.a1 = r.qa; c.b0 = p.b0; c.b1 = r.qb;
                    iv[slot] = c; best[slot] = 0; wmax[slot] = 0; depth[slot] = dp + 1; res[slot] = nr;
                    if (danger) { dg.best[slot] = 0; dg.flag[slot] = 0; dg.ceil[slot] = 0; }
                    r.lead = slot;
                } else atomicOr(&counters[C_ERR], 1u);
                slot++;
            }
            if (trail) {
                if (slot < child_cap) {
                    CasIv c; c.a0 = (sa_t)((int64_t)r.qa + r.ql); c.a1 = p.a1; c.b0 = (sa_t)((int64_t)r.qb + r.ql); c.b1 = p.b1;
                    iv[slot] = c; best[slot] = 0; wmax[slot] = 0; depth[slot] = dp + 1; res[slot] = nr;
                    if (danger) { dg.best[slot] = 0; dg.flag[slot] = 0; dg.ceil[slot] = 0; }
                    r.trail = slot;
                } else atomicOr(&counters[C_ERR], 1u);
            }
            const u32 as = base_a + (u32)__popcll(b_split & lt);
            if (as < io.anchor_cap) { io.anchor_l[as] = r.ql; io.anchor_pos[2 * (size_t)as] = (int64_t)r.qa; io.anchor_pos[2 * (size_t)as + 1] = (int64_t)r.qb; }
            else atomicOr(&counters[C_ERR], 4u);
            r.state = 1;
        } else {
            r.state = 2;
        }
        if (in) res[id] = r;
        if (und) {
            und_list[base_u + (u32)__popcll(b_und & lt)] = id;
            if ((u64)(la + lb) > (u64)leaf_n) atomicMax(&counters[C_MAXN], (u32)((la + lb) > 0xFFFFFFFFll ? 0xFFFFFFFFll : (la + lb)));
        }
        __syncthreads();
    }
    if (threadIdx.x == 0) {
        __threadfence();
        if (atomicAdd(&counters[C_TICKET], 1u) == gridDim.x - 1) {
            if (hi > lo) counters[C_LEVELS]++;
            counters[C_LO] = hi; counters[C_HI] = atomicAdd(&counters[C_NCHILD], 0u);
            counters[C_NANCH] = atomicAdd(io.anchor_count, 0u);
            counters[C_TICKET] = 0;
        }
    }
}
__global__ __launch_bounds__(TB) void k_cas_stats(const u32 *__restrict__ counters, const int32_t *__restrict__ depth, RvCascadeIO io) {
    __shared__ unsigned long long s_bp[TB / 64];
    __shared__ u32 s_md[TB / 64];
    const u32 nchild = counters[C_NCHILD], na = *io.anchor_count;
    unsigned long long bp = 0; u32 md = 0;
    for (u32 i = blockIdx.x * TB + threadIdx.x; i < na; i += gridDim.x * TB) bp += io.anchor_l[i];
    for (u32 i = blockIdx.x * TB + threadIdx.x; i < nchild; i += gridDim.x * TB) { const u32 d = (u32)depth[i]; md = d > md ? d : md; }
#pragma unroll
    for (int d = 32; d >= 1; d >>= 1) {
        bp += ((unsigned long long)(u32)__shfl_down((u32)(bp >> 32), d, 64) << 32) + (unsigned long long)(u32)__shfl_down((u32)bp, d, 64);
        const u32 om = __shfl_down(md, d, 64);
        md = om > md ? om : md;
    }
    if ((threadIdx.x & 63) == 0) { s_bp[threadIdx.x >> 6] = bp; s_md[threadIdx.x >> 6] = md; }
    __syncthreads();
    if (threadIdx.x == 0) {
        for (int k = 1; k < TB / 64; k++) { bp += s_bp[k]; md = s_md[k] > md ? s_md[k] : md; }
        if (bp) atomicAdd(&io.stats[2], bp);
        if (md) atomicMax(&io.stats[3], (unsigned long long)md);
        if (blockIdx.x == 0) { atomicAdd(&io.stats[0], (unsigned long long)(nchild - counters[C_NUND] - counters[C_NRETRY])); atomicAdd(&io.stats[1], (unsigned long long)na); }
    }
}

__global__ __launch_bounds__(TB) void k_cas_sizes(const u32 *__restrict__ und_list, u32 U, const CasIv *__restrict__ iv, u64 *__restrict__ sizes) {
    const u32 u = blockIdx.x * TB + threadIdx.x;
    if (u < U) { const CasIv p = iv[und_list[u]]; sizes[u] = (u64)(((int64_t)p.a1 - p.a0) + ((int64_t)p.b1 - p.b0)); }
    if (u == U) sizes[u] = 0;
}
__global__ __launch_bounds__(TB) void k_cas_roots(const u32 *__restrict__ und_list, u32 U, const CasIv *__restrict__ iv, const int32_t *__restrict__ depth,
                                                  const u64 *__restrict__ offs, RvLeafRoot *__restrict__ roots) {
    const u32 u = blockIdx.x * TB + threadIdx.x;
    if (u >= U) return;
    const u32 id = und_list[u];
    const CasIv p = iv[id];
    RvLeafRoot r;
    r.off = (int64_t)offs[u]; r.n = (int32_t)(((int64_t)p.a1 - p.a0) + ((int64_t)p.b1 - p.b0)); r.depth = depth[id];
    r.a0 = p.a0; r.a1 = p.a1; r.b0 = p.b0; r.b1 = p.b1;
    roots[u] = r;
}

constexpr int BN = RV_LEAF_N;
__device__ inline int cas_first_diff(const uint8_t *txt, int i, int j, int lim) {
    int x = 0;
    while (x + 8 <= lim) {
        u64 a, b;
        __builtin_memcpy(&a, txt + i + x, 8);
        __builtin_memcpy(&b, txt + j + x, 8);
        if (a != b) return x + (__builtin_ctzll(a ^ b) >> 3);
        x += 8;
    }
// ... 184 lines not shown
                 oL = put(rootLead.data(), (size_t)P * 4), oT = put(rootTrail.data(), (size_t)P * 4);
    RV_TRY(btabs.reserve(o + 64));
    RV_HIP(hipMemcpyAsync(btabs.p, stage.data(), o, hipMemcpyHostToDevice, q));
    if (R) {
        RV_HIP(hipMemcpyAsync(broots.p, roots.data(), (size_t)R * sizeof(CasIv), hipMemcpyHostToDevice, q));
        RV_HIP(hipMemcpyAsync(bdepth.p, rdepth.data(), (size_t)R * 4, hipMemcpyHostToDevice, q));
    }
    RV_HIP(hipMemcpyAsync(banch.p, anp.data(), (size_t)P * 16, hipMemcpyHostToDevice, q));
    RV_HIP(hipMemcpyAsync((uint8_t *)banch.p + (size_t)P * 16, anl.data(), (size_t)P * 4, hipMemcpyHostToDevice, q));
    RV_HIP(hipStreamSynchronize(q));
    cb.lin_roots = R; cb.lin_picks = P; cb.lin_nA = (u32)nA; cb.lin_nB = (u32)nB; cb.lin_steps = steps; cb.lin_maxdepth = maxdepth;
    cb.lin_off[0] = oA; cb.lin_off[1] = oB; cb.lin_off[2] = opA; cb.lin_off[3] = opB; cb.lin_off[4] = oL; cb.lin_off[5] = oT;
    return 0;
}

int rv_cascade_run(rv_index *h, RvCascadeBufs &cb, const RvCascadeIO &io, int minl_in, RvCascadeOut *out, int danger, int reuse, const RvCascadeHost *host) {
    memset(out, 0, sizeof *out);
    out->done = false;
    Workspace &ws = h->ws;
    hipStream_t q = ws.stream;
    const int64_t n = h->n;
    const u32 minl = (u32)std::max(minl_in, 1);
    const bool verbose = (ws.opt.cascade_log != 0);
    double tp[6] = {0, 0, 0, 0, 0, 0};
    if (verbose) { (void)hipStreamSynchronize(q); tp[0] = cas_now(); }
#define GIVE_UP(msg) do { out->why = msg; if (verbose) fprintf(stderr, "cascade: gave up: %s\n", msg); return 0; } while (0)
    if (h->nsamples != 2 || h->nsep.size() != 1 || h->nodes.size() < 2) GIVE_UP("not two samples");
    std::vector<RvIntv> CA, CB;
    for (const RvIntv &v : h->nodes) if (v.end > v.begin) (v.begin < h->nsep[0] ? CA : CB).push_back(v);
    std::sort(CA.begin(), CA.end(), [](const RvIntv &x, const RvIntv &y) { return x.begin < y.begin; });
    std::sort(CB.begin(), CB.end(), [](const RvIntv &x, const RvIntv &y) { return x.begin < y.begin; });
    if (CA.empty() || CB.empty()) GIVE_UP("an empty sample");
    const bool chain = CA.size() > 1 || CB.size() > 1;
    if (chain && ws.opt.no_cascade_chain) GIVE_UP("several sequences per sample (switched off)");
    if (n >= ((int64_t)1 << 32) - 2) GIVE_UP("index above 2^32 positions");
#ifdef RV_SA64
    if ((u64)h->maxlcp >= (1ull << 24) || n >= ((int64_t)1 << 40)) GIVE_UP("bid word too narrow");
#endif
    CasIv root; root.a0 = root.a1 = root.b0 = root.b1 = 0;
    root.a0 = (sa_t)CA[0].begin; root.a1 = (sa_t)CA[0].end; root.b0 = (sa_t)CB[0].begin; root.b1 = (sa_t)CB[0].end;
    if (root.a0 >= root.a1 || root.b0 >= root.b1 || (int64_t)root.a1 > h->nsep[0] || (int64_t)root.b0 <= h->nsep[0]) GIVE_UP("an empty sample");

    const sa_t *SA = h->dSA.as<sa_t>(); const lcp_t *LCP = h->dLCP.as<lcp_t>(); const uint8_t *BWT = h->dBWT.as<uint8_t>();

    const int64_t ntile = ceil_div(n, RV_PAIR_TILE);
    DBuf &bcnt = ws.misc[14], &btab = ws.misc[2], &bslot = ws.misc[3], &bovf = ws.misc[4], &bout = ws.misc[5];
    if (bcnt.cap == 0) { RV_TRY(bcnt.reserve(64)); RV_HIP(hipMemsetAsync(bcnt.p, 0, 64, q)); }
    RV_TRY(btab.reserve((size_t)(ntile + 1) * 3 * sizeof(u32)));
    RV_TRY(bslot.reserve((size_t)ntile * RV_PAIR_SLOTS * sizeof(RvPairRec)));
    if (bovf.cap < 4096 * sizeof(RvPairRec)) RV_TRY(bovf.reserve(4096 * sizeof(RvPairRec)));
    if (bout.cap < 4096 * sizeof(RvPairRec)) RV_TRY(bout.reserve(sizeof(RvPairRec) * (size_t)std::max<int64_t>(4096, n / 64)));
    u32 *tilecnt = btab.as<u32>(), *tileovf = tilecnt + (ntile + 1), *tileoff = tileovf + (ntile + 1);
    u32 M = reuse ? cb.M : 0;
    for (int attempt = 0; !reuse; attempt++) {
        if (attempt == 3) { rv_set_error("cascade: scan buffer sizing failed"); return -1; }
        const size_t ocap = bout.cap / sizeof(RvPairRec) - RV_PAIR_HDR, vcap = bovf.cap / sizeof(RvPairRec);
        hipEvent_t ev_a, ev_b;
        (void)h->prof.attach(RV_K_SCAN_PAIR, (double)n * 8.0, &ev_a, &ev_b);
        RV_TRY(rv_scan_pair_launch(ws, SA, LCP, n, BWT, (sa_t)h->nsep[0], (int)minl, bslot.as<RvPairRec>(), bovf.as<RvPairRec>(),
                                   (u32)std::min<size_t>(vcap, 0xffffffffu), bcnt.as<u32>(), tilecnt, tileovf, nullptr, nullptr, 0, ev_a, ev_b));
        RV_TRY(rv_exclusive_sum_u32(ws, tilecnt, tileoff, ntile + 1));
        RV_TRY(rv_pair_compact_launch(ws, bslot.as<RvPairRec>(), bovf.as<RvPairRec>(), tilecnt, tileovf, tileoff, ntile, bout.as<RvPairRec>(),
                                      (u32)std::min<size_t>(ocap, 0xffffffffu), bcnt.as<u32>(), nullptr, (u32)std::min<size_t>(vcap, 0xffffffffu)));
        u32 hdr[4];
        RV_TRY(rv_read_back(ws, hdr, bout.p, sizeof hdr));
        const u32 total = hdr[0], novf = hdr[1];
        if (total <= ocap && novf <= vcap) { M = total; break; }
        if (novf > vcap) RV_TRY(bovf.reserve((size_t)novf * sizeof(RvPairRec)));
        if (total > ocap) RV_TRY(bout.reserve(((size_t)total + RV_PAIR_HDR) * sizeof(RvPairRec)));
    }
    if (verbose) tp[1] = cas_now();
    out->cands = M;
    struct ProfSpan { Workspace &w; int id; ~ProfSpan() { w.prof_end(id); } } span{ws, ws.prof_begin(RV_K_CASCADE, 5.0 * (double)n)};
    if (M == 0) GIVE_UP("no match at the top level");
    const RvPairRec *recs = bout.as<RvPairRec>() + RV_PAIR_HDR;
    cb.M = M;

    const int64_t rcap64 = std::min<int64_t>(n / WT_REGIONS + WT_TILE, std::max<int64_t>(16384, n / 1024));
    const u32 wcap = (u32)std::min<int64_t>(rcap64 * WT_REGIONS, 0x7fffffff);
    const int64_t ccap64 = n / (int64_t)minl + 16;
    if (ccap64 >= 0x7fffffff) GIVE_UP("too many sub-indices possible");
    const u32 ccap = (u32)ccap64;
    DBuf &k0 = cb.d[0], &k1 = cb.d[1], &v0 = cb.d[2], &v1 = cb.d[3], &bpa = cb.d[4], &bpb = cb.d[5], &blen = cb.d[6], &bcc = cb.d[7], &bwp = cb.d[8], &bwv = cb.d[9],
         &bwc = cb.d[10], &biv = cb.d[11], &bbest = cb.d[12], &bwm = cb.d[13], &bdep = cb.d[14], &bres = cb.d[15], &bctr = cb.d[16], &bund = cb.d[17], &bsz = cb.d[18];
    RV_TRY(k0.reserve((size_t)M * 8)); RV_TRY(k1.reserve((size_t)M * 8)); RV_TRY(v0.reserve((size_t)M * 4)); RV_TRY(v1.reserve((size_t)M * 4));
    RV_TRY(bpa.reserve((size_t)M * sizeof(sa_t))); RV_TRY(bpb.reserve((size_t)M * sizeof(sa_t))); RV_TRY(blen.reserve((size_t)M * 4)); RV_TRY(bcc.reserve((size_t)M * 4));
    RV_TRY(bwp.reserve((size_t)wcap * sizeof(sa_t))); RV_TRY(bwv.reserve((size_t)wcap * 4)); RV_TRY(bwc.reserve((size_t)wcap * 4));
    RV_TRY(biv.reserve((size_t)ccap * sizeof(CasIv))); RV_TRY(bbest.reserve((size_t)ccap * 8)); RV_TRY(bwm.reserve((size_t)ccap * 4)); RV_TRY(bdep.reserve((size_t)ccap * 4));
    RV_TRY(bres.reserve((size_t)ccap * sizeof(CasRes))); RV_TRY(bctr.reserve(64)); RV_TRY(bund.reserve((size_t)ccap * 4));
    u32 *counters = bctr.as<u32>();
    RV_HIP(hipMemsetAsync(counters, 0, 64, q));

    DBuf &bwp0 = cb.d[19], &bwv0 = cb.d[20], &bwr = cb.d[21], &bwrk = cb.d[22], &bwrk0 = cb.d[23];
    RV_TRY(bwp0.reserve((size_t)wcap * sizeof(sa_t))); RV_TRY(bwv0.reserve((size_t)wcap * 4)); RV_TRY(bwr.reserve(2 * WT_REGIONS * 4 + 64));
    RV_TRY(bwrk.reserve((size_t)wcap * 4)); RV_TRY(bwrk0.reserve((size_t)wcap * 4));
    u32 hc[16];
    u32 NW = reuse ? cb.NW : 0;
    if (!reuse) {
        u32 *wreg = bwr.as<u32>();
        RV_HIP(hipMemsetAsync(wreg, 0, 2 * WT_REGIONS * 4, q));
        const u32 wrcap = wcap / WT_REGIONS;
        hipLaunchKernelGGL(k_cas_witness, dim3((unsigned)ceil_div(n, WT_TILE)), dim3(TB), 0, q, SA, LCP, BWT, n, minl, bwp0.as<sa_t>(), bwv0.as<u32>(), bwrk0.as<u32>(), wrcap, wreg);
        RV_LAUNCH_CHECK();
        {
            const unsigned mb = (unsigned)ceil_div((int64_t)M, TB);
            hipLaunchKernelGGL(k_cas_keys, dim3(mb), dim3(TB), 0, q, recs, M, k0.as<u64>(), v0.as<u32>());
            RV_LAUNCH_CHECK();
            int in1 = 0;
            RV_TRY(rv_radix_sort_pairs<u32>(ws, k0.as<u64>(), v0.as<u32>(), k1.as<u64>(), v1.as<u32>(), (int64_t)M, 0, bitlen64((u64)n), &in1));
            hipLaunchKernelGGL(k_cas_gather, dim3(mb), dim3(TB), 0, q, recs, (const u32 *)(in1 ? v1.as<u32>() : v0.as<u32>()), M, bpa.as<sa_t>(), bpb.as<sa_t>(),
                               blen.as<u32>(), bcc.as<u32>());
            RV_LAUNCH_CHECK();
        }
        u32 hreg[2 * WT_REGIONS];
        RV_TRY(rv_read_back(ws, hreg, wreg, WT_REGIONS * 4));
        u32 wmaxc = 0;
        for (int r = 0; r < WT_REGIONS; r++) { hreg[WT_REGIONS + r] = NW; NW += hreg[r]; wmaxc = std::max(wmaxc, hreg[r]); }
        out->witnesses = NW;
        if (wmaxc > wrcap) GIVE_UP("too many repeat witnesses (a repetitive input)");
        if (NW) {
            RV_HIP(hipMemcpyAsync(wreg + WT_REGIONS, hreg + WT_REGIONS, WT_REGIONS * 4, hipMemcpyHostToDevice, q));
            RV_HIP(hipStreamSynchronize(q));
            hipLaunchKernelGGL(k_cas_wpack, dim3((unsigned)std::max<int64_t>(1, ceil_div((int64_t)wmaxc, TB)), WT_REGIONS), dim3(TB), 0, q, (const sa_t *)bwp0.as<sa_t>(),
                               (const u32 *)bwv0.as<u32>(), (const u32 *)bwrk0.as<u32>(), wrcap, (const u32 *)wreg, (const u32 *)(wreg + WT_REGIONS), bwp.as<sa_t>(), bwv.as<u32>(),
                               bwrk.as<u32>());
            RV_LAUNCH_CHECK();
        }
        cb.NW = NW;
        if (chain) {
            const char *why = nullptr;
            RV_TRY(cas_lineage(h, cb, M, NW, minl, CA, CB, &why));
            if (why) { cb.lin_picks = 0; cb.lin_rest.clear(); GIVE_UP(why); }
        }
    } else {
        if (chain && cb.lin_picks == 0) GIVE_UP("the chain of rest sub-indices was not decided");
        RV_HIP(hipMemsetAsync(bcc.p, 0, (size_t)M * 4, q));
        out->witnesses = NW;
    }
    const sa_t *wp = bwp.as<sa_t>(); const u32 *wv = bwv.as<u32>();
    CasDanger dg; memset(&dg, 0, sizeof dg);
    u32 dwalk_nmed = 0; const u32 *dwalk_boff = nullptr, *dwalk_mlist = nullptr;
    if (danger) {
        if (NW) {
            RV_TRY(k0.reserve((size_t)NW * 8)); RV_TRY(k1.reserve((size_t)NW * 8)); RV_TRY(v0.reserve((size_t)NW * 4)); RV_TRY(v1.reserve((size_t)NW * 4));
            const unsigned wb = (unsigned)ceil_div((int64_t)NW, TB);
            hipLaunchKernelGGL(k_cas_wkeys, dim3(wb), dim3(TB), 0, q, (const u32 *)bwrk.as<u32>(), NW, k0.as<u64>(), v0.as<u32>());
            RV_LAUNCH_CHECK();
            int in1 = 0;
            RV_TRY(rv_radix_sort_pairs<u32>(ws, k0.as<u64>(), v0.as<u32>(), k1.as<u64>(), v1.as<u32>(), (int64_t)NW, 0, bitlen64((u64)n), &in1));
            hipLaunchKernelGGL(k_cas_wgather, dim3(wb), dim3(TB), 0, q, (const sa_t *)bwp.as<sa_t>(), (const u32 *)bwv.as<u32>(), (const u32 *)(in1 ? v1.as<u32>() : v0.as<u32>()), NW,
                               bwp0.as<sa_t>(), bwv0.as<u32>());
            RV_LAUNCH_CHECK();
            wp = bwp0.as<sa_t>(); wv = bwv0.as<u32>();
            dg.rank = in1 ? k1.as<u64>() : k0.as<u64>();
        }
        DBuf &bdc = cb.d[24], &bdw = cb.d[25];
        const size_t per_child = 8 + 8 + 4 + sizeof(sa_t) + 1, per_wit = 4 + 4 + 4 + 8;
        RV_TRY(bdc.reserve((size_t)ccap * per_child + 64)); RV_TRY(bdw.reserve((size_t)std::max<u32>(NW, 1) * per_wit + 64));
        dg.best = bdc.as<u64>(); dg.ceil = dg.best + ccap; dg.qb = (sa_t *)(dg.ceil + ccap); dg.flag = (u32 *)(dg.qb + ccap); dg.dflag = (uint8_t *)(dg.flag + ccap);
        dg.key = bdw.as<u64>(); dg.m1 = (u32 *)(dg.key + std::max<u32>(NW, 1)); dg.p1 = dg.m1 + std::max<u32>(NW, 1); dg.m2 = dg.p1 + std::max<u32>(NW, 1);
        dg.T0 = h->dT0.as<uint8_t>(); dg.LCP = LCP;
        if (NW && !ws.opt.no_dwalk_blocks) {
            DBuf &bfl = cb.d[35], &bbid = cb.d[36], &bboff = cb.d[37], &bml = cb.d[38], &bwcls = cb.d[39];
            RV_TRY(bfl.reserve((size_t)(NW + 1) * 4)); RV_TRY(bbid.reserve((size_t)(NW + 1) * 4)); RV_TRY(bwcls.reserve((size_t)NW + 16));
            const unsigned wb = (unsigned)ceil_div((int64_t)NW, TB);
            hipLaunchKernelGGL(k_cas_blk_flags, dim3(wb), dim3(TB), 0, q, dg.rank, LCP, NW, minl, bfl.as<u32>());
            RV_LAUNCH_CHECK();
            RV_HIP(hipMemsetAsync(bfl.as<u32>() + NW, 0, 4, q));
            RV_TRY(rv_exclusive_sum_u32(ws, bfl.as<u32>(), bbid.as<u32>(), (int64_t)NW + 1));
            u32 nb = 0;
            RV_TRY(rv_read_back(ws, &nb, bbid.as<u32>() + NW, 4));
            RV_TRY(bboff.reserve((size_t)(nb + 2) * 4)); RV_TRY(bml.reserve((size_t)(nb + 2) * 4 * 3));
            u32 *mflag = bml.as<u32>(), *mid = mflag + (nb + 1), *mlist = mid + (nb + 1);
            hipLaunchKernelGGL(k_cas_blk_off, dim3(wb), dim3(TB), 0, q, (const u32 *)bfl.as<u32>(), (const u32 *)bbid.as<u32>(), NW, nb, bboff.as<u32>());
            RV_LAUNCH_CHECK();
            hipLaunchKernelGGL(k_cas_blk_class, dim3(wb), dim3(TB), 0, q, (const u32 *)bfl.as<u32>(), (const u32 *)bbid.as<u32>(), (const u32 *)bboff.as<u32>(), NW, mflag, bwcls.as<uint8_t>());
            RV_LAUNCH_CHECK();
            RV_HIP(hipMemsetAsync(mflag + nb, 0, 4, q));
            RV_TRY(rv_exclusive_sum_u32(ws, mflag, mid, (int64_t)nb + 1));
            RV_TRY(rv_read_back(ws, &dwalk_nmed, mid + nb, 4));
            if (dwalk_nmed) {
                hipLaunchKernelGGL(k_cas_blk_list, dim3((unsigned)ceil_div((int64_t)nb, TB)), dim3(TB), 0, q, (const u32 *)mflag, (const u32 *)mid, nb, mlist);
                RV_LAUNCH_CHECK();
                dg.wcls = bwcls.as<uint8_t>();
                dwalk_boff = bboff.as<u32>(); dwalk_mlist = mlist;
            }
        }
        dg.leaf_n = (u32)ws.opt.cascade_danger_min;
    }
    const sa_t *d_beginA = nullptr, *d_beginB = nullptr;
    if (!chain) {
        hipLaunchKernelGGL(k_cas_init, dim3((unsigned)std::max<int64_t>(1, ceil_div((int64_t)NW, TB))), dim3(TB), 0, q, biv.as<CasIv>(), bbest.as<u64>(), bwm.as<u32>(),
                           bdep.as<int32_t>(), bres.as<CasRes>(), counters, root, bwc.as<u32>(), NW, dg.best, dg.flag, dg.ceil);
        RV_LAUNCH_CHECK();
    } else {
        const u32 R = cb.lin_roots, P = cb.lin_picks;
        if ((int64_t)R + 16 > (int64_t)ccap || P > io.anchor_cap) GIVE_UP("more sequences than the cascade's tables hold");
        const uint8_t *tb = cb.d[32].as<uint8_t>();
        CasRootTabs rt;
        rt.beginA = (const sa_t *)(tb + cb.lin_off[0]); rt.beginB = (const sa_t *)(tb + cb.lin_off[1]);
        rt.pickA = (const int32_t *)(tb + cb.lin_off[2]); rt.pickB = (const int32_t *)(tb + cb.lin_off[3]);
        rt.rootLead = (const u32 *)(tb + cb.lin_off[4]); rt.rootTrail = (const u32 *)(tb + cb.lin_off[5]);
        rt.nA = cb.lin_nA; rt.nB = cb.lin_nB;
        d_beginA = rt.beginA; d_beginB = rt.beginB;
        hipLaunchKernelGGL(k_cas_init_roots, dim3((unsigned)std::max<int64_t>(1, ceil_div((int64_t)R, TB))), dim3(TB), 0, q, biv.as<CasIv>(), bbest.as<u64>(), bwm.as<u32>(),
                           bdep.as<int32_t>(), bres.as<CasRes>(), counters, (const CasIv *)cb.d[30].as<CasIv>(), (const int32_t *)cb.d[31].as<int32_t>(), R, dg.best, dg.flag, dg.ceil);
        RV_LAUNCH_CHECK();
        hipLaunchKernelGGL(k_cas_assign_roots, dim3((unsigned)std::max<int64_t>(1, ceil_div((int64_t)std::max(M, NW), TB))), dim3(TB), 0, q, (const sa_t *)bpa.as<sa_t>(),
                           (const sa_t *)bpb.as<sa_t>(), (const u32 *)blen.as<u32>(), bcc.as<u32>(), M, wp, bwc.as<u32>(), NW, (const CasIv *)cb.d[30].as<CasIv>(), rt, (int64_t)minl);
        RV_LAUNCH_CHECK();
        RV_HIP(hipMemcpyAsync(io.anchor_pos, cb.d[33].p, (size_t)P * 16, hipMemcpyDeviceToDevice, q));
        RV_HIP(hipMemcpyAsync(io.anchor_l, (const uint8_t *)cb.d[33].p + (size_t)P * 16, (size_t)P * 4, hipMemcpyDeviceToDevice, q));
        RV_HIP(hipMemcpyAsync(io.anchor_count, &cb.lin_picks, 4, hipMemcpyHostToDevice, q));
    }

    if (verbose) { (void)hipStreamSynchronize(q); tp[2] = cas_now(); }
    const unsigned agrid = (unsigned)(ceil_div((int64_t)M, TB * CAS_ITEMS) + ceil_div((int64_t)NW, TB * CAS_ITEMS));
    const int batch = std::max(1, (int)ws.opt.cascade_batch);
    int queued = 0;
    RV_TRY(rv_working_text_begin(h, host ? host->side : nullptr));
    u32 sent = 0, known = 0;
    auto send_known = [&]() -> int {
        if (!host || !host->side || !host->l || known <= sent || known > host->cap) return 0;
        RV_HIP(hipMemcpyAsync(host->pos + 2 * (size_t)sent, io.anchor_pos + 2 * (size_t)sent, (size_t)(known - sent) * 16, hipMemcpyDeviceToHost, host->side));
        RV_HIP(hipMemcpyAsync(host->l + sent, io.anchor_l + sent, (size_t)(known - sent) * 4, hipMemcpyDeviceToHost, host->side));
        sent = known;
        return 0;
    };
    struct PrioScope {
        Workspace &w; hipStream_t home; RvCascadeBufs &cb; bool on = false;
        ~PrioScope() { leave(); }
        void leave() {
            if (!on) return;
            on = false;
            (void)hipEventRecord(cb.ev_out, w.stream);
            w.stream = home;
            (void)hipStreamWaitEvent(home, cb.ev_out, 0);
        }
    } prio{ws, q, cb};
    if (ws.opt.cascade_prio) {
        if (!cb.prio_stream) {
            int plo = 0, phi = 0;
            RV_HIP(hipDeviceGetStreamPriorityRange(&plo, &phi));
            RV_HIP(hipStreamCreateWithPriority(&cb.prio_stream, hipStreamNonBlocking, phi));
            RV_HIP(hipEventCreateWithFlags(&cb.ev_in, hipEventDisableTiming));
            RV_HIP(hipEventCreateWithFlags(&cb.ev_out, hipEventDisableTiming));
        }
        RV_HIP(hipEventRecord(cb.ev_in, q));
        RV_HIP(hipStreamWaitEvent(cb.prio_stream, cb.ev_in, 0));
        ws.stream = cb.prio_stream; prio.on = true;
        q = cb.prio_stream;
    }
    for (;;) {
        for (int b = 0; b < batch; b++, queued++) {
            hipLaunchKernelGGL(k_cas_assign, dim3(agrid), dim3(TB), 0, q, (const sa_t *)bpa.as<sa_t>(), (const sa_t *)bpb.as<sa_t>(), (const u32 *)blen.as<u32>(), bcc.as<u32>(), M,
                               wp, wv, bwc.as<u32>(), NW, (const CasIv *)biv.as<CasIv>(), (const CasRes *)bres.as<CasRes>(),
                               bbest.as<u64>(), bwm.as<u32>(), (int64_t)minl, queued == 0 ? 1 : 0, (const u64 *)((danger && NW) ? dg.ceil : nullptr));
            RV_LAUNCH_CHECK();
            hipLaunchKernelGGL(k_cas_winner, dim3((unsigned)ceil_div((int64_t)M, TB)), dim3(TB), 0, q, (const sa_t *)bpa.as<sa_t>(), (const sa_t *)bpb.as<sa_t>(),
                               (const u32 *)blen.as<u32>(), (const u32 *)bcc.as<u32>(), M, (const CasIv *)biv.as<CasIv>(), bres.as<CasRes>(), (const u64 *)bbest.as<u64>(), (int64_t)minl);
            RV_LAUNCH_CHECK();
            if (danger && NW) {
                const unsigned wb = (unsigned)ceil_div((int64_t)NW, TB);
                hipLaunchKernelGGL(k_cas_dmark, dim3(256), dim3(TB), 0, q, (const CasIv *)biv.as<CasIv>(), (const u64 *)bbest.as<u64>(), (const u32 *)bwm.as<u32>(), minl, (const u32 *)counters, dg);
                RV_LAUNCH_CHECK();
                hipLaunchKernelGGL(k_cas_dwalk, dim3(wb), dim3(TB), 0, q, wp, wv, (const u32 *)bwc.as<u32>(), NW, (const CasIv *)biv.as<CasIv>(), (const u64 *)bbest.as<u64>(),
                                   (const u32 *)bwm.as<u32>(), minl, dg);
                RV_LAUNCH_CHECK();
                if (dwalk_nmed) {
                    hipLaunchKernelGGL(k_cas_dwalk_blk, dim3((unsigned)dwalk_nmed), dim3(TB), 0, q, wp, wv, (const u32 *)bwc.as<u32>(), dwalk_boff, dwalk_mlist, dwalk_nmed,
                                       (const CasIv *)biv.as<CasIv>(), (const u64 *)bbest.as<u64>(), (const u32 *)bwm.as<u32>(), minl, dg);
                    RV_LAUNCH_CHECK();
                }
                hipLaunchKernelGGL(k_cas_dpick, dim3(wb), dim3(TB), 0, q, wp, wv, (const u32 *)bwc.as<u32>(), NW, (const CasIv *)biv.as<CasIv>(), (const CasRes *)bres.as<CasRes>(),
                                   (const u64 *)bbest.as<u64>(), (const u32 *)bwm.as<u32>(), minl, dg);
                RV_LAUNCH_CHECK();
                hipLaunchKernelGGL(k_cas_dwrite, dim3(wb), dim3(TB), 0, q, wp, (const u32 *)bwc.as<u32>(), NW, dg);
                RV_LAUNCH_CHECK();
            }
            hipLaunchKernelGGL(k_cas_decide, dim3(256), dim3(TB), 0, q, biv.as<CasIv>(), bbest.as<u64>(), bwm.as<u32>(), bdep.as<int32_t>(),
                               bres.as<CasRes>(), minl, counters, ccap, bund.as<u32>(), (u32)RV_LEAF_N, io, dg, (danger && NW) ? 1 : 0);
            RV_LAUNCH_CHECK();
        }
        RV_TRY(send_known());
        RV_TRY(rv_read_back(ws, hc, counters, sizeof hc));
        if (hc[C_ERR] & ~5u) { rv_set_error("cascade: device error %u", hc[C_ERR]); return -1; }
        if (hc[C_ERR]) GIVE_UP("the cascade's tables are full");
        known = hc[C_NANCH];
        if (hc[C_MAXN] > (u32)RV_LEAF_N) break;
        if (hc[C_HI] == hc[C_LO]) break;
        if (queued > 1000000) { rv_set_error("cascade: no progress"); return -1; }
    }
    prio.leave(); q = ws.stream;
    const int level = (int)hc[C_LEVELS];
    const u32 hi = hc[C_NCHILD];
    if (verbose) tp[3] = cas_now();
    out->levels = level; out->children = hi; out->solved = hc[C_NSOLVED]; out->unsolved = hc[C_NUNSOLVED];
    const u32 U = hc[C_NUND];
    out->undecided = U;
    if (hc[C_MAXN] > (u32)RV_LEAF_N) {
        out->why = "an undecided sub-index above the leaf kernel's size";
        if (verbose) fprintf(stderr, "cascade%s: gave up: %s (%u ranks; %u levels, %u sub-indices, %u undecided, %u decided from witnesses, %u not)\n", danger ? " (second attempt)" : "", out->why, hc[C_MAXN], level, hi, U, hc[C_NSOLVED], hc[C_NUNSOLVED]);
        return 0;
    }
    hipLaunchKernelGGL(k_cas_stats, dim3(256), dim3(TB), 0, q, (const u32 *)counters, (const int32_t *)bdep.as<int32_t>(), io);
    RV_LAUNCH_CHECK();
    RV_TRY(send_known());
    if (chain) {
        hipLaunchKernelGGL(k_cas_lineage_stats, dim3(1), dim3(64), 0, q, io.stats, (unsigned long long)cb.lin_steps, (unsigned long long)cb.lin_maxdepth);
        RV_LAUNCH_CHECK();
    }
    if (U > 0) {
        RV_TRY(bsz.reserve((size_t)(U + 1) * 8));
        u64 *sizes = bsz.as<u64>();
        hipLaunchKernelGGL(k_cas_sizes, dim3((unsigned)ceil_div((int64_t)U + 1, TB)), dim3(TB), 0, q, (const u32 *)bund.as<u32>(), U, (const CasIv *)biv.as<CasIv>(), sizes);
        RV_LAUNCH_CHECK();
        RV_TRY(rv_exclusive_sum_u64(ws, sizes, sizes, (int64_t)U + 1));
        u64 mu = 0;
        RV_TRY(rv_read_back(ws, &mu, sizes + U, 8));
        out->rebuilt_ranks = (int64_t)mu;
        RV_TRY(io.lvSA->reserve((size_t)(mu + 64) * sizeof(sa_t))); RV_TRY(io.lvLCP->reserve((size_t)(mu + 64) * sizeof(lcp_t))); RV_TRY(io.lvBWT->reserve((size_t)mu + 64));
        RV_TRY(io.roots->reserve((size_t)U * sizeof(RvLeafRoot)));
        RvLeafRoot *roots = io.roots->as<RvLeafRoot>();
        hipLaunchKernelGGL(k_cas_roots, dim3((unsigned)ceil_div((int64_t)U, TB)), dim3(TB), 0, q, (const u32 *)bund.as<u32>(), U, (const CasIv *)biv.as<CasIv>(),
                           (const int32_t *)bdep.as<int32_t>(), (const u64 *)sizes, roots);
        RV_LAUNCH_CHECK();
        DBuf &bord = cb.d[26];
        RV_TRY(bord.reserve((size_t)(mu + 64) * 2));
        hipLaunchKernelGGL(k_cas_rank, dim3(U, BN / TB), dim3(TB), 0, q, (const RvLeafRoot *)roots, (const uint8_t *)h->dT0.as<uint8_t>(), bord.as<uint16_t>());
        RV_LAUNCH_CHECK();
        hipLaunchKernelGGL(k_cas_emit, dim3(U, BN / TB), dim3(TB), 0, q, (const RvLeafRoot *)roots, (const uint8_t *)h->dT0.as<uint8_t>(), (const uint16_t *)bord.as<uint16_t>(),
                           io.lvSA->as<sa_t>(), io.lvLCP->as<lcp_t>(), io.lvBWT->as<uint8_t>(), h->nsep[0], (int64_t)root.a0, (int64_t)root.b0,
                           d_beginA, cb.lin_nA, d_beginB, cb.lin_nB);
        RV_LAUNCH_CHECK();
        RvLeafArgs la;
        la.roots = roots;
        la.SA = io.lvSA->as<sa_t>(); la.LCP = io.lvLCP->as<lcp_t>(); la.BWT = io.lvBWT->as<uint8_t>();
        la.nsep0 = h->nsep[0]; la.minl = minl_in; la.lcap = h->maxlcp;
        la.stage_cap = io.stage_cap;
        la.anchor_count = io.anchor_count; la.anchor_cap = io.anchor_cap; la.anchor_l = io.anchor_l; la.anchor_pos = io.anchor_pos;
        la.stats = io.stats;
        la.trace = 0; la.trace_count = io.anchor_count + 1; la.trace_cap = 0; la.trace_out = nullptr;
        la.err = io.leaf_err;
        RV_TRY(rv_leaf_launch(ws, la, (int)U));
    }
    if (verbose) {
        (void)hipStreamSynchronize(q); tp[4] = cas_now();
        fprintf(stderr, "cascade%s: %u matches, %u witnesses, %d levels, %u sub-indices, %u undecided (%lld ranks rebuilt), %lld decided from witnesses | ms: scan %.2f witnesses+sort %.2f levels %.2f rebuild+leaf %.2f\n",
                danger ? " (second attempt)" : "", M, NW, level, hi, U, (long long)out->rebuilt_ranks, (long long)out->solved, (tp[1] - tp[0]) * 1e3, (tp[2] - tp[1]) * 1e3, (tp[3] - tp[2]) * 1e3, (tp[4] - tp[3]) * 1e3);
    }
    out->done = true;
    out->sent = sent;
    return 0;
#undef GIVE_UP
}
```

reveal_amd/csrc/rv_cascade_multi.hip:

```cpp
#include "rv_index.h"
#include "rv_cascade.h"
#include "rv_leaf.h"
#include <algorithm>
#include <chrono>
#include <condition_variable>
#include <mutex>
#include <string.h>
#include <stdio.h>
#include <stdlib.h>

namespace {

constexpr int TB = 256;
constexpr u32 NONE = 0xFFFFFFFFu;
#ifdef RV_SA64
constexpr int KEY_SHIFT = 40;
#else
constexpr int KEY_SHIFT = 32;
#endif
constexpr u64 KEY_LOW = (1ull << KEY_SHIFT) - 1;
enum { C_NCHILD = 0, C_NUND = 1, C_NWIT = 2, C_ERR = 3, C_MAXN = 4, C_LO = 5, C_HI = 6, C_LEVELS = 7, C_NCAND = 8, C_NANCH = 9, C_STEPS = 10, C_MAXDEPTH = 11, C_TICKET = 12, C_BIGERR = 13, C_BIGTOT = 14  };

__device__ inline int cm_sample(const sa_t *__restrict__ nsep, int k, sa_t pos) {
    int s = 0;
// ... 951 lines not shown
    RV_TRY(bcl.reserve((size_t)M * 4)); RV_TRY(bcp.reserve((size_t)M * k * sizeof(sa_t))); RV_TRY(bcc.reserve((size_t)M * 4));
    RV_TRY(bwp.reserve((size_t)(NW + 1) * sizeof(sa_t))); RV_TRY(bwv.reserve((size_t)(NW + 1) * 4)); RV_TRY(bwc.reserve((size_t)(NW + 1) * 4)); RV_TRY(bws.reserve((size_t)NW + 64));
    const size_t per = (size_t)3 * k * sizeof(sa_t) + 8 + 7 * 4;
    RV_TRY(btb.reserve(per * ccap + 256)); RV_TRY(bctr.reserve(256)); RV_TRY(bund.reserve((size_t)ccap * 4));
    RV_TRY(banl.reserve((size_t)acap * 4)); RV_TRY(banp.reserve((size_t)acap * k * sizeof(sa_t)));
    RV_TRY(bst.reserve((size_t)J * 16 + 64));
    CmTabs t;
    {
        uint8_t *p = btb.as<uint8_t>();
        t.best = (u64 *)p; p += (size_t)ccap * 8;
        t.b = (sa_t *)p; p += (size_t)ccap * k * sizeof(sa_t); t.e = (sa_t *)p; p += (size_t)ccap * k * sizeof(sa_t); t.q = (sa_t *)p; p += (size_t)ccap * k * sizeof(sa_t);
        t.rmax = (u32 *)p; p += (size_t)ccap * 4; t.depth = (int32_t *)p; p += (size_t)ccap * 4; t.state = (u32 *)p; p += (size_t)ccap * 4;
        t.lead = (u32 *)p; p += (size_t)ccap * 4; t.trail = (u32 *)p; p += (size_t)ccap * 4; t.ql = (u32 *)p; p += (size_t)ccap * 4; t.job = (u32 *)p;
    }
    g->t = t;
    const size_t o_m = 0, o_w = o_m + ((size_t)J + 1) * 4, o_rb = (o_w + ((size_t)J + 1) * 4 + 15) & ~(size_t)15, o_re = o_rb + (size_t)J * k * sizeof(sa_t),
                 o_sep = o_re + (size_t)J * k * sizeof(sa_t), o_ab = (o_sep + (size_t)J * (k - 1) * sizeof(sa_t) + 15) & ~(size_t)15, sm_bytes = o_ab + ((size_t)J + 1) * 4 + 64;
    RV_TRY(g->hs.reserve(sm_bytes)); RV_TRY(bsm.reserve(sm_bytes));
    uint8_t *hp = g->hs.as<uint8_t>();
    memset(hp, 0, sm_bytes);
    memcpy(hp + o_m, moff.data(), ((size_t)J + 1) * 4); memcpy(hp + o_w, woff.data(), ((size_t)J + 1) * 4);
    for (int j = 0; j < J; j++) {
        memcpy(hp + o_rb + (size_t)j * k * sizeof(sa_t), jobs[(size_t)j]->rb.data(), (size_t)k * sizeof(sa_t));
        memcpy(hp + o_re + (size_t)j * k * sizeof(sa_t), jobs[(size_t)j]->re.data(), (size_t)k * sizeof(sa_t));
        memcpy(hp + o_sep + (size_t)j * (k - 1) * sizeof(sa_t), jobs[(size_t)j]->sep.data(), (size_t)(k - 1) * sizeof(sa_t));
    }
    std::vector<u32> abase((size_t)J + 1, 0);
    for (int j = 0; j < J; j++) abase[(size_t)j + 1] = abase[(size_t)j] + jobs[(size_t)j]->acap;
    memcpy(hp + o_ab, abase.data(), ((size_t)J + 1) * 4);
    DBuf &bjc = g->d[16];
    RV_TRY(bjc.reserve((size_t)J * 256 + 64));
    RV_HIP(hipMemsetAsync(bjc.p, 0, (size_t)J * 256, q));
    uint8_t *dsm = bsm.as<uint8_t>();
    RV_HIP(hipMemcpyAsync(dsm, hp, sm_bytes, hipMemcpyHostToDevice, q));
    u32 *counters = bctr.as<u32>();
    for (int j = 0; j < J; j++) {
        RvBatchJob &x = *jobs[(size_t)j];
        RV_HIP(hipStreamWaitEvent(q, x.ready, 0));
        if (x.M) {
            RV_HIP(hipMemcpyAsync(bcl.as<u32>() + moff[(size_t)j], x.c_len, (size_t)x.M * 4, hipMemcpyDeviceToDevice, q));
            RV_HIP(hipMemcpyAsync(bcp.as<sa_t>() + (size_t)moff[(size_t)j] * k, x.c_pos, (size_t)x.M * k * sizeof(sa_t), hipMemcpyDeviceToDevice, q));
        }
        if (x.NW) {
            RV_HIP(hipMemcpyAsync(bwp.as<sa_t>() + woff[(size_t)j], x.w_pos, (size_t)x.NW * sizeof(sa_t), hipMemcpyDeviceToDevice, q));
            RV_HIP(hipMemcpyAsync(bwv.as<u32>() + woff[(size_t)j], x.w_val, (size_t)x.NW * 4, hipMemcpyDeviceToDevice, q));
        }
    }
    hipLaunchKernelGGL(k_cmj_fill, dim3((unsigned)ceil_div((int64_t)std::max(M, NW), TB)), dim3(TB), 0, q, M, NW, (const u32 *)(dsm + o_m), (const u32 *)(dsm + o_w), J, k,
                       (const sa_t *)(dsm + o_sep), (const sa_t *)bwp.as<sa_t>(), bcc.as<u32>(), bwc.as<u32>(), bws.as<uint8_t>());
    RV_LAUNCH_CHECK();
    hipLaunchKernelGGL(k_cmj_init, dim3((unsigned)ceil_div((int64_t)J, 64)), dim3(64), 0, q, t, k, (const sa_t *)(dsm + o_rb), (const sa_t *)(dsm + o_re), J, counters);
    RV_LAUNCH_CHECK();
    const unsigned agrid = (unsigned)(ceil_div((int64_t)M, TB) + ceil_div((int64_t)NW, TB));
    const int batch = std::max(1, (int)ws.opt.cascade_batch);
    const u32 big_min = (u32)std::min<int64_t>(jobs[0]->big_min, 0x7fffffff);
    u32 hc[16];
    int queued = 0;
    for (;;) {
        for (int b = 0; b < batch; b++, queued++) {
            hipLaunchKernelGGL(k_casm_assign, dim3(agrid), dim3(TB), 0, q, (const sa_t *)bcp.as<sa_t>(), (const u32 *)bcl.as<u32>(), bcc.as<u32>(), M, (const sa_t *)bwp.as<sa_t>(),
                               (const u32 *)bwv.as<u32>(), bwc.as<u32>(), NW, t, k, (const sa_t *)nullptr, (int64_t)minl, queued == 0 ? 1 : 0, (const uint8_t *)bws.as<uint8_t>());
            RV_LAUNCH_CHECK();
            hipLaunchKernelGGL(k_casm_winner, dim3((unsigned)ceil_div((int64_t)M, TB)), dim3(TB), 0, q, (const sa_t *)bcp.as<sa_t>(), (const u32 *)bcl.as<u32>(), (const u32 *)bcc.as<u32>(), M, t, k,
                               (int64_t)minl);
            RV_LAUNCH_CHECK();
            hipLaunchKernelGGL(k_casm_decide, dim3(192), dim3(TB), 0, q, t, k, minl, counters, ccap, bund.as<u32>(), big_min, banl.as<u32>(), banp.as<sa_t>(), acap, (u32 *)nullptr,
                               bjc.as<u32>(), (const u32 *)(dsm + o_ab));
            RV_LAUNCH_CHECK();
        }
        RV_TRY(rv_read_back(ws, hc, counters, sizeof hc));
        if (hc[C_ERR]) return 0;
        if (hc[C_HI] == hc[C_LO]) break;
        if (queued > 1000000) return 0;
    }
    const u32 NCH = hc[C_NCHILD], U = hc[C_NUND];
    RV_HIP(hipMemsetAsync(bst.p, 0, (size_t)J * 16, q));
    hipLaunchKernelGGL(k_cmj_stats, dim3((unsigned)ceil_div((int64_t)NCH, TB)), dim3(TB), 0, q, t, NCH, bst.as<u32>());
    RV_LAUNCH_CHECK();
    const size_t rowbytes = (size_t)U * 12 + (size_t)U * k * sizeof(sa_t) * 2;
    const size_t h_st = 0, h_jc = ((size_t)J * 16 + 15) & ~(size_t)15, h_rows = h_jc + (size_t)J * 256;
    RV_TRY(g->hs2.reserve(h_rows + rowbytes + 64));
    uint8_t *h2 = g->hs2.as<uint8_t>();
    RV_HIP(hipMemcpyAsync(h2 + h_st, bst.p, (size_t)J * 16, hipMemcpyDeviceToHost, q));
    RV_HIP(hipMemcpyAsync(h2 + h_jc, bjc.p, (size_t)J * 256, hipMemcpyDeviceToHost, q));
    if (U) {
        RV_TRY(brows.reserve(rowbytes + 64));
        u32 *d_id = brows.as<u32>(); int32_t *d_dep = (int32_t *)(d_id + U); u32 *d_job = (u32 *)(d_dep + U);
        sa_t *d_b = (sa_t *)(d_job + U), *d_e = d_b + (size_t)U * k;
        hipLaunchKernelGGL(k_cmj_rows, dim3((unsigned)ceil_div((int64_t)U * k, TB)), dim3(TB), 0, q, (const u32 *)bund.as<u32>(), U, t, k, d_id, d_dep, d_job, d_b, d_e);
        RV_LAUNCH_CHECK();
        RV_HIP(hipMemcpyAsync(h2 + h_rows, brows.p, rowbytes, hipMemcpyDeviceToHost, q));
    }
    RV_HIP(hipStreamSynchronize(q));
    const u32 *st = (const u32 *)(h2 + h_st), *jc = (const u32 *)(h2 + h_jc);
    for (int j = 0; j < J; j++) {
        RvBatchJob &x = *jobs[(size_t)j];
        x.nchild = st[(size_t)j * 4]; x.levels = st[(size_t)j * 4 + 1] + 1; x.maxdepth = st[(size_t)j * 4 + 2];
        x.na = jc[(size_t)j * 64];
        if (x.na > x.acap) return 0;
        x.d_anl = banl.as<u32>() + abase[(size_t)j]; x.d_anp = banp.as<sa_t>() + (size_t)abase[(size_t)j] * k;
        x.und_id.clear(); x.und_dep.clear(); x.und_b.clear(); x.und_e.clear(); x.too_big = false; x.maxn = 0;
    }
    std::vector<unsigned long long> bigtot((size_t)J, 0);
    if (U) {
        const u32 *r_id = (const u32 *)(h2 + h_rows); const int32_t *r_dep = (const int32_t *)(r_id + U); const u32 *r_job = (const u32 *)(r_dep + U);
        const sa_t *r_b = (const sa_t *)(r_job + U), *r_e = r_b + (size_t)U * k;
        for (u32 u2 = 0; u2 < U; u2++) {
// ... 150 lines not shown
    };
    bool joint = false;
    RvBatchJob bjob;
    if (h->batch && !h->batch_settled) {
        h->batch_settled = true; ticket.settled = true;
        bjob.k = k; bjob.minl = minl; bjob.M = M; bjob.NW = std::min(NW, wcap); bjob.ccap = ccap; bjob.acap = acap;
        bjob.c_len = bcl.as<u32>(); bjob.c_pos = bcp.as<sa_t>(); bjob.w_pos = bwp.as<sa_t>(); bjob.w_val = bwv.as<u32>();
        bjob.nsep = nsep; bjob.dT = h->dT.as<uint8_t>();
        bjob.rb = rb; bjob.re = re;
        for (int s2 = 0; s2 + 1 < k; s2++) bjob.sep.push_back((sa_t)h->nsep[(size_t)s2]);
        bjob.big_min = big_min; bjob.big_root = ws.opt.casm_big_root; bjob.big_total = ws.opt.casm_big_total; bjob.no_big = no_big;
        bjob.stream = q;
        if (!cb.ev_in) RV_HIP(hipEventCreateWithFlags(&cb.ev_in, hipEventDisableTiming));
        bjob.ready = cb.ev_in;
        RV_HIP(hipEventRecord(cb.ev_in, q));
        batch_join(h->batch, &bjob, ws);
        joint = bjob.ok;
        if (joint) {
            RV_HIP(hipStreamWaitEvent(q, h->batch->ev_done, 0));
            t = h->batch->t;
            memset(hc, 0, sizeof hc);
            hc[C_LEVELS] = bjob.levels; hc[C_NCHILD] = bjob.nchild; hc[C_NUND] = (u32)bjob.und_id.size(); hc[C_NANCH] = bjob.na;
            hc[C_STEPS] = bjob.steps; hc[C_MAXDEPTH] = bjob.maxdepth; hc[C_MAXN] = bjob.maxn;
        }
    }
    if (!joint) {
    struct PrioScope {
        Workspace &w; hipStream_t home; RvCascadeBufs &cb; bool on = false;
        ~PrioScope() { leave(); }
        void leave() {
            if (!on) return;
            on = false;
            (void)hipEventRecord(cb.ev_out, w.stream);
            w.stream = home;
            (void)hipStreamWaitEvent(home, cb.ev_out, 0);
        }
    } prio{ws, q, cb};
    if (ws.opt.cascade_prio) {
        if (!cb.prio_stream) {
            int lo = 0, hi = 0;
            RV_HIP(hipDeviceGetStreamPriorityRange(&lo, &hi));
            RV_HIP(hipStreamCreateWithPriority(&cb.prio_stream, hipStreamNonBlocking, hi));
            RV_HIP(hipEventCreateWithFlags(&cb.ev_in, hipEventDisableTiming));
            RV_HIP(hipEventCreateWithFlags(&cb.ev_out, hipEventDisableTiming));
        }
        RV_HIP(hipEventRecord(cb.ev_in, q));
        RV_HIP(hipStreamWaitEvent(cb.prio_stream, cb.ev_in, 0));
        ws.stream = cb.prio_stream; prio.on = true;
        q = cb.prio_stream;
    }
    hipLaunchKernelGGL(k_casm_init, dim3((unsigned)std::max<int64_t>(1, ceil_div((int64_t)NW, TB))), dim3(TB), 0, q, t, k, d_rb, d_re, counters, bwc.as<u32>(), NW);
    RV_LAUNCH_CHECK();
    const unsigned agrid = (unsigned)(ceil_div((int64_t)M, TB) + ceil_div((int64_t)NW, TB));
    const int batch = std::max(1, (int)ws.opt.cascade_batch);
    int queued = 0;
    for (;;) {
        for (int b = 0; b < batch; b++, queued++) {
            hipLaunchKernelGGL(k_casm_assign, dim3(agrid), dim3(TB), 0, q, (const sa_t *)bcp.as<sa_t>(), (const u32 *)bcl.as<u32>(), bcc.as<u32>(), M, (const sa_t *)bwp.as<sa_t>(),
                               (const u32 *)bwv.as<u32>(), bwc.as<u32>(), NW, t, k, nsep, (int64_t)minl, queued == 0 ? 1 : 0);
            RV_LAUNCH_CHECK();
            hipLaunchKernelGGL(k_casm_winner, dim3((unsigned)ceil_div((int64_t)M, TB)), dim3(TB), 0, q, (const sa_t *)bcp.as<sa_t>(), (const u32 *)bcl.as<u32>(), (const u32 *)bcc.as<u32>(), M, t, k,
                               (int64_t)minl);
            RV_LAUNCH_CHECK();
            hipLaunchKernelGGL(k_casm_decide, dim3(192), dim3(TB), 0, q, t, k, minl, counters, ccap, bund.as<u32>(), (u32)big_min, banl.as<u32>(), banp.as<sa_t>(), acap);
            RV_LAUNCH_CHECK();
        }
        RV_TRY(rv_read_back(ws, hc, counters, sizeof hc));
        if (hc[C_ERR] & ~5u) { rv_set_error("cascade (multi): device error %u", hc[C_ERR]); return -1; }
        if (hc[C_ERR]) GIVE_UP("the cascade's tables are full");
        if (too_big(hc)) break;
        if (hc[C_HI] == hc[C_LO]) break;
        if (queued > 1000000) { rv_set_error("cascade (multi): no progress"); return -1; }
    }
    prio.leave(); q = ws.stream;
    }
    out->levels = (int)hc[C_LEVELS]; out->children = hc[C_NCHILD];
    const u32 U = hc[C_NUND], NA = hc[C_NANCH];
    out->undecided = U;
    if (joint ? bjob.too_big : too_big(hc)) {
        out->why = "an undecided sub-index above the size that is rebuilt from the text";
        if (verbose) fprintf(stderr, "cascade (%d samples): gave up: %s (%u ranks; %u levels, %u sub-indices, %u undecided)\n", k, out->why, hc[C_MAXN], hc[C_LEVELS], hc[C_NCHILD], U);
        return 0;
    }
    if (U == 1 && hc[C_NCHILD] == 1 && n > (int64_t)BN)
        GIVE_UP("the index' longest match of all samples is no longer than its repeats");
    out->steps = hc[C_STEPS]; out->maxdepth = (int)hc[C_MAXDEPTH];
    const size_t b_anl = 0, b_anp = b_anl + (((size_t)NA * 4 + 15) & ~(size_t)15), b_rows = b_anp + (((size_t)NA * k * sizeof(sa_t) + 15) & ~(size_t)15);
    const size_t rowbytes = (size_t)U * 8 + (size_t)U * k * sizeof(sa_t) * 2;
    RV_TRY(cb.hstage.reserve(b_rows + rowbytes + 64));
    uint8_t *hs = cb.hstage.as<uint8_t>();
    const u32 *d_anl = joint ? bjob.d_anl : (const u32 *)banl.as<u32>();
    const sa_t *d_anp = joint ? bjob.d_anp : (const sa_t *)banp.as<sa_t>();
    if (joint) {
        if (NA) {
            RV_HIP(hipMemcpyAsync(hs + b_anl, d_anl, (size_t)NA * 4, hipMemcpyDeviceToHost, q));
            RV_HIP(hipMemcpyAsync(hs + b_anp, d_anp, (size_t)NA * k * sizeof(sa_t), hipMemcpyDeviceToHost, q));
        }
        if (U) {
            uint8_t *hr = hs + b_rows;
            memcpy(hr, bjob.und_id.data(), (size_t)U * 4); memcpy(hr + (size_t)U * 4, bjob.und_dep.data(), (size_t)U * 4);
            memcpy(hr + (size_t)U * 8, bjob.und_b.data(), (size_t)U * k * sizeof(sa_t)); memcpy(hr + (size_t)U * 8 + (size_t)U * k * sizeof(sa_t), bjob.und_e.data(), (size_t)U * k * sizeof(sa_t));
        }
    } else {
    if (NA) {
        RV_HIP(hipMemcpyAsync(hs + b_anl, banl.p, (size_t)NA * 4, hipMemcpyDeviceToHost, q));
        RV_HIP(hipMemcpyAsync(hs + b_anp, banp.p, (size_t)NA * k * sizeof(sa_t), hipMemcpyDeviceToHost, q));
        RV_TRY(bexp.reserve((size_t)NA * k * 4));
// ... 127 lines not shown
```

reveal_amd/csrc/rv_common.h:

```cpp
#pragma once
#include <mutex>
#include <thread>
#include <vector>
#include <utility>
#include <hip/hip_runtime.h>
#include <stdint.h>
#include <string.h>
#include <stddef.h>
#include <vector>
#include <string>

#ifdef RV_SA64
typedef int64_t  sa_t;
typedef uint32_t lcp_t;
#else
typedef int32_t  sa_t;
typedef int32_t  lcp_t;
#endif

typedef unsigned long long u64;
typedef unsigned int       u32;

void rv_set_error(const char *fmt, ...);

#define RV_HIP(x)                                                                              \
    do {                                                                                       \
        hipError_t e_ = (x);                                                                   \
        if (e_ != hipSuccess) {                                                                \
            rv_set_error("%s:%d %s: %s", __FILE__, __LINE__, #x, hipGetErrorString(e_));       \
            return -1;                                                                         \
        }                                                                                      \
    } while (0)
#define RV_TRY(x)                                                                              \
    do {                                                                                       \
        int r_ = (x);                                                                          \
        if (r_ != 0) return r_;                                                                \
    } while (0)
#define RV_OPTION_LIST(X) \
    X(bubble_par_min, "RV_BUBBLE_PAR_MIN", -1) \
    X(presel_log, "RV_PRESEL_LOG", 0) \
    X(presel_host, "RV_PRESEL_HOST", 0) \
    X(leaf_acap, "RV_LEAF_ACAP", 256) \
    X(bubble_lds_always, "RV_BUBBLE_LDS_ALWAYS", 0) \
    X(no_early_bubble, "RV_NO_EARLY_BUBBLE", 0) \
    X(early_bubble_many, "RV_EARLY_BUBBLE_MANY", 0) \
    X(no_early_split, "RV_NO_EARLY_SPLIT", 0) \
    X(keep_dead, "RV_KEEP_DEAD", 0) \
    X(bubble_no_lds, "RV_BUBBLE_NO_LDS", 0) \
    X(bubble_no_join, "RV_BUBBLE_NO_JOIN", 0) \
    X(bubble_no_merge, "RV_BUBBLE_NO_MERGE", 0) \
    X(tables_memcpy, "RV_TABLES_MEMCPY", 0) \
    X(bubble_parent_scratch, "RV_BUBBLE_PARENT_SCRATCH", 0) \
    X(level_log, "RV_LEVEL_LOG", 0) \
    X(pb_two_pass, "RV_PB_TWO_PASS", 0) \
    X(no_leaf, "RV_NO_LEAF", 0) \
    X(leaf_prof, "RV_LEAF_PROF", 0) \
    X(no_cascade, "RV_NO_CASCADE", 0) \
    X(cascade_second, "RV_CASCADE_SECOND", 0) \
    X(cascade_danger, "RV_CASCADE_DANGER", 1) \
    X(cascade_second_off, "RV_CASCADE_SECOND_OFF", 0) \
    X(sync_block, "RV_SYNC_BLOCK", 0) \
    X(pb_refresh_tmin, "RV_PB_REFRESH_TMIN", 0) \
    X(cascade_log, "RV_CASCADE_LOG", 0) \
    X(cascade_danger_min, "RV_CASCADE_DANGER_MIN", 0) \
    X(cascade_batch, "RV_CASCADE_BATCH", 8) \
    X(lcp_by_rank, "RV_LCP_BY_RANK", 0) \
    X(no_tiny_sa, "RV_NO_TINY_SA", 0) \
    X(no_short_alphabet, "RV_NO_SHORT_ALPHABET", 0) \
    X(no_fused_lcp, "RV_NO_FUSED_LCP", 0) \
    X(no_diag, "RV_NO_DIAG", 0) \
    X(no_packed_text, "RV_NO_PACKED_TEXT", 0) \
    X(no_heads_fusion, "RV_NO_HEADS_FUSION", 0) \
    X(no_twin_collapse, "RV_NO_TWIN_COLLAPSE", 0) \
    X(no_far_twins, "RV_NO_FAR_TWINS", 0) \
    X(no_lcp_list, "RV_NO_LCP_LIST", 0) \
    X(no_text_jump, "RV_NO_TEXT_JUMP", 0) \
    X(far_table, "RV_FAR_TABLE", 0) \
    X(no_slow_class, "RV_NO_SLOW_CLASS", 0) \
    X(no_dwalk_blocks, "RV_NO_DWALK_BLOCKS", 0) \
    X(no_pub_twins, "RV_NO_PUB_TWINS", 0) \
    X(sa_no_text, "RV_SA_NO_TEXT", 0) \
    X(text_mode, "RV_TEXT_MODE", -1) \
    X(carry_ch, "RV_CARRY_CH", -1) \
    X(rs_bits, "RV_RS_BITS", 8) \
    X(rs_xcd, "RV_RS_XCD", 1) \
    X(rs_cnt16, "RV_RS_CNT16", 1) \
    X(rs_no_digit_bytes, "RV_RS_NO_DIGIT_BYTES", 0) \
    X(diag_table, "RV_DIAG_TABLE", -1) \
    X(no_cascade_chain, "RV_NO_CASCADE_CHAIN", 0) \
    X(casm_rank_count, "RV_CASM_RANK_COUNT", 0) \
    X(casm_big_min, "RV_CASM_BIG_MIN", -1) \
    X(casm_no_big, "RV_CASM_NO_BIG", 0) \
    X(casm_big_root, "RV_CASM_BIG_ROOT", 1 << 22) \
    X(casm_big_total, "RV_CASM_BIG_TOTAL", 1 << 26) \
    X(lock_any, "RV_LOCK_ANY", 0) \
    X(presel_dev_min, "RV_PRESEL_DEV_MIN", 65536) \
    X(scan_v1, "RV_SCAN_V1", 0) \
    X(pick_threads, "RV_PICK_THREADS", 0) \
    X(cascade_prio, "RV_CASCADE_PRIO", 0)
struct RvOptions {
#define RV_X_(f, name, def) int64_t f = def;
    RV_OPTION_LIST(RV_X_)
#undef RV_X_
    int64_t *find(const char *name) {
#define RV_X_(f, nm, def) if (strcmp(name, nm) == 0) return &f;
        RV_OPTION_LIST(RV_X_)
#undef RV_X_
        return nullptr;
    }
};
extern int g_rv_launch_trace;
static inline bool rv_launch_trace_on() { return g_rv_launch_trace != 0; }
#define RV_LAUNCH_CHECK()                                                                      \
    do {                                                                                       \
        RV_HIP(hipGetLastError());                                                             \
        if (rv_launch_trace_on()) {                                                            \
            fprintf(stderr, "launch %s:%d\n", __FILE__, __LINE__);                             \
            fflush(stderr);                                                                    \
// ... 238 lines not shown
```

Before: 23920.

## Overlap cascade tail: double-buffered counter landing, side-stream witness pass, background offset fill

```diff
diff --git a/include/reveal_amd.h b/include/reveal_amd.h
--- a/include/reveal_amd.h
+++ b/include/reveal_amd.h
@@ -88,6 +88,7 @@
 int rv_frontier_seeds_import(rv_index *h, int nsubs, const int64_t *words, int64_t nwords);
 uint32_t rv_maxlcp(const rv_index *h);
 int rv_cascade_info(const rv_index *h, int64_t *out);
+int rv_cascade_tail_info(const rv_index *h, int64_t out[4]);
 const char *rv_cascade_why(const rv_index *h);
 int64_t rv_anchor_count(rv_index *h, int64_t *members);
 int rv_fetch_anchors(rv_index *h, uint32_t *l, int64_t *off, int64_t *pos);
diff --git a/reveal_amd/_index.py b/reveal_amd/_index.py
--- a/reveal_amd/_index.py
+++ b/reveal_amd/_index.py
@@ -599,7 +599,10 @@
         def cascade_info(self):
             o = np.zeros(8, dtype=np.int64)
             self._dll.rv_cascade_info(self._h, o.ctypes.data)
-            return dict(done=bool(o[0]), levels=int(o[1]), matches=int(o[2]), witnesses=int(o[3]), subindices=int(o[4]), undecided=int(o[5]), rebuilt_ranks=int(o[6]), decided_from_witnesses=int(o[7]),
+            t = np.zeros(4, dtype=np.int64)
+            self._dll.rv_cascade_tail_info(self._h, t.ctypes.data)
+            return dict(lowered_early=int(t[0]), offsets_early=int(t[1]), batches_ahead=int(t[2]), witness_on_side=bool(t[3]),
+                        done=bool(o[0]), levels=int(o[1]), matches=int(o[2]), witnesses=int(o[3]), subindices=int(o[4]), undecided=int(o[5]), rebuilt_ranks=int(o[6]), decided_from_witnesses=int(o[7]),
                         why=(self._dll.rv_cascade_why(self._h) or b"").decode())
 
         def align_builtin_until(self, stop_subs, minl=20, minn=2, trace=False):
diff --git a/reveal_amd/_lib.py b/reveal_amd/_lib.py
--- a/reveal_amd/_lib.py
+++ b/reveal_amd/_lib.py
@@ -79,6 +79,7 @@
     "rv_maxlcp": (ctypes.c_uint32, [V]),
     "rv_cascade_info": (ctypes.c_int, [V, V]),
     "rv_cascade_why": (ctypes.c_char_p, [V]),
+    "rv_cascade_tail_info": (ctypes.c_int, [V, V]),
     "rv_anchor_count": (_L, [V, c_i64p]),
     "rv_fetch_anchors": (_I, [V, V, V, V]),
     "rv_set_result_buffers": (_I, [V, V, _L, V, _L, V, _L]),
diff --git a/reveal_amd/csrc/rv_align.hip b/reveal_amd/csrc/rv_align.hip
--- a/reveal_amd/csrc/rv_align.hip
+++ b/reveal_amd/csrc/rv_align.hip
@@ -190,6 +190,7 @@
     bool running = false;
     u32 *lf_counters = nullptr; unsigned long long *lf_stats = nullptr; u32 *lf_l = nullptr; int64_t *lf_pos = nullptr; rv_trace *lf_tr = nullptr;
     size_t early_sent = 0; u32 *early_l = nullptr; int64_t *early_pos = nullptr;
+    size_t early_filled = 0; int64_t *early_off = nullptr;
     size_t leaf_na = 0;
     void release() {
         if (leaf_stream) (void)hipStreamSynchronize(leaf_stream);
@@ -1415,7 +1416,7 @@
     RV_TRY(align_begin(h, minl, minn, h->al && h->al->trace_on));
     Align *a = h->al;
     a->full_only = !a->trace_on && a->picker == 0;
-    a->an_l.clear(); a->an_off.assign(1, 0); a->an_pos.clear(); a->trace.clear(); a->leaf_na = 0; a->early_sent = 0;
+    a->an_l.clear(); a->an_off.assign(1, 0); a->an_pos.clear(); a->trace.clear(); a->leaf_na = 0; a->early_sent = 0; a->early_filled = 0;
     a->seeds_cur.clear(); a->seeds_lead.clear(); a->seeds_trail.clear(); a->picker_calls = a->picker_seeded = 0; a->picker_ns = a->picker_list_ns = a->galign_ns = 0;
     if (a->picker == 1) {
         if ((int)h->nodes.size() != h->nsamples) { rv_set_error("the native picker (rv_set_picker) takes one sequence per sample: %d sequences in %d samples", (int)h->nodes.size(), h->nsamples); return -1; }
@@ -1834,14 +1835,16 @@
             int64_t *pp; u32 *pl;
             if (rb.direct) { pp = rb.pos + np; pl = rb.l + nl; }
             else { RV_TRY(a->hLeafOut.reserve(na * 20 + 64)); pp = a->hLeafOut.as<int64_t>(); pl = (u32 *)(pp + 2 * na); }
-            const size_t sent = (rb.direct && a->early_l == pl && a->early_pos == pp) ? std::min(a->early_sent, na) : 0;
+            const bool same = rb.direct && a->early_l == pl && a->early_pos == pp;
+            const size_t sent = same ? std::min(a->early_sent, na) : 0;
+            const size_t filled = (same && a->early_off == rb.off + nl + 1) ? std::min(a->early_filled, na) : 0;
             if (sent < na) {
                 RV_HIP(hipMemcpyAsync(pp + 2 * sent, lf_pos + 2 * sent, (na - sent) * 16, hipMemcpyDeviceToHost, a->leaf_stream));
                 RV_HIP(hipMemcpyAsync(pl + sent, lf_l + sent, (na - sent) * 4, hipMemcpyDeviceToHost, a->leaf_stream));
             }
             RV_TRY(rv_ensure_working_text(h));
             RV_TRY(rv_leaf_lower_launch(h->ws, h->dT.as<uint8_t>(), lf_pos, lf_l, (u32)na));
-            if (rb.direct) fill_offsets(rb.off + nl + 1, na, (int64_t)np);
+            if (rb.direct) fill_offsets(rb.off + nl + 1 + filled, na - filled, (int64_t)(np + 2 * filled));
             RV_HIP(hipStreamSynchronize(a->leaf_stream));
             RV_HIP(hipStreamSynchronize(q));
             a->leaf_na = na;
@@ -1904,11 +1907,12 @@
     io.stage_cap = (u32)h->ws.opt.leaf_acap;
     RvCascadeHost hx;
     hx.side = a->leaf_stream;
-    a->early_sent = 0;
+    a->early_sent = 0; a->early_filled = 0;
+    for (int k = 0; k < 4; k++) a->cas.tail[k] = 0;
     if (h->rb.l) {
         const int64_t nl = (int64_t)a->an_l.size(), np = (int64_t)a->an_pos.size();
         const int64_t room = std::min(std::min(h->rb.l_cap - nl, h->rb.off_cap - nl - 1), (h->rb.pos_cap - np) / 2);
-        if (room > 0) { hx.l = h->rb.l + nl; hx.pos = h->rb.pos + np; hx.cap = (u32)std::min<int64_t>(room, 0xffffffffll); }
+        if (room > 0) { hx.l = h->rb.l + nl; hx.pos = h->rb.pos + np; hx.cap = (u32)std::min<int64_t>(room, 0xffffffffll); hx.off = h->rb.off + nl + 1; hx.off_base = np; }
     }
     io.lvSA = &a->lvSA[0]; io.lvLCP = &a->lvLCP[0]; io.lvBWT = &a->lvBWT[0]; io.roots = &a->dLeafRoots[0];
     const int dmode = (int)h->ws.opt.cascade_danger;
@@ -1926,6 +1930,7 @@
     a->st.levels += a->cas_out.levels;
     a->st.scanned_ranks += h->n;
     a->early_sent = a->cas_out.sent; a->early_l = hx.l; a->early_pos = hx.pos;
+    a->early_filled = a->cas_out.filled; a->early_off = hx.off;
     if (!a->cas.lin_rest.empty() && h->nodes.size() > 2) {
         std::vector<RvIntv> rest, gone;
         for (size_t k = 0; k + 1 < a->cas.lin_rest.size(); k += 2) rest.push_back({a->cas.lin_rest[k], a->cas.lin_rest[k + 1]});
@@ -1952,6 +1957,11 @@
     if (!h->al) return 0;
     const RvCascadeOut &c = h->al->cas_out;
     out[0] = c.done ? 1 : 0; out[1] = c.levels; out[2] = c.cands; out[3] = c.witnesses; out[4] = c.children; out[5] = c.undecided; out[6] = c.rebuilt_ranks; out[7] = c.solved;
+    return 0;
+}
+
+int rv_cascade_tail_info(const rv_index *h, int64_t *out) {
+    for (int k = 0; k < 4; k++) out[k] = h->al ? h->al->cas.tail[k] : 0;
     return 0;
 }
 
@@ -2135,7 +2145,7 @@
             if (h->rc) { rv_set_error("the native picker (rv_set_picker) with construct(rc=1) is not supported"); return -1; }
         }
         a->picker_calls = a->picker_seeded = 0; a->picker_ns = a->picker_list_ns = a->galign_ns = 0;
-        a->an_l.clear(); a->an_off.assign(1, 0); a->an_pos.clear(); a->trace.clear(); a->leaf_na = 0; a->early_sent = 0;
+        a->an_l.clear(); a->an_off.assign(1, 0); a->an_pos.clear(); a->trace.clear(); a->leaf_na = 0; a->early_sent = 0; a->early_filled = 0;
         RV_TRY(builtin_leaf_setup(h));
     }
     RV_TRY(install_frontier(h, level, nsubs, meta, node_first, nodes, m, sa, lcp, bwt, on_device));
diff --git a/reveal_amd/csrc/rv_cascade.h b/reveal_amd/csrc/rv_cascade.h
--- a/reveal_amd/csrc/rv_cascade.h
+++ b/reveal_amd/csrc/rv_cascade.h
@@ -10,8 +10,12 @@
     int64_t lin_steps = 0; int lin_maxdepth = 0; size_t lin_off[6] = {0, 0, 0, 0, 0, 0};
     std::vector<int64_t> lin_rest; int lin_rest_depth = 0;
     hipStream_t prio_stream = nullptr; hipEvent_t ev_in = nullptr, ev_out = nullptr;
+    hipEvent_t ev_scan = nullptr, ev_wit = nullptr, ev_land[2] = {nullptr, nullptr};
+    HBuf hland;
+    int64_t tail[4] = {0, 0, 0, 0};
     void release() {
-        for (auto &b : d) b.release(); hstage.release(); hstage2.release();
+        for (auto &b : d) b.release(); hstage.release(); hstage2.release(); hland.release();
+        for (hipEvent_t *e : {&ev_scan, &ev_wit, &ev_land[0], &ev_land[1]}) if (*e) { (void)hipEventDestroy(*e); *e = nullptr; }
         if (prio_stream) { (void)hipStreamDestroy(prio_stream); prio_stream = nullptr; }
         if (ev_in) { (void)hipEventDestroy(ev_in); ev_in = nullptr; }
         if (ev_out) { (void)hipEventDestroy(ev_out); ev_out = nullptr; }
@@ -29,6 +33,7 @@
 struct RvCascadeHost {
     hipStream_t side = nullptr;
     int64_t *pos = nullptr; u32 *l = nullptr; u32 cap = 0;
+    int64_t *off = nullptr; int64_t off_base = 0;
 };
 
 struct RvCascadeOut {
@@ -38,6 +43,7 @@
     int64_t solved, unsolved;
     const char *why;
     u32 sent;
+    u32 filled;
 };
 
 #define RV_CASM_K 16
diff --git a/reveal_amd/csrc/rv_cascade.hip b/reveal_amd/csrc/rv_cascade.hip
--- a/reveal_amd/csrc/rv_cascade.hip
+++ b/reveal_amd/csrc/rv_cascade.hip
@@ -6,6 +6,8 @@
 #include <stdio.h>
 #include <stdlib.h>
 #include <chrono>
+#include <atomic>
+#include <thread>
 
 namespace {
 
@@ -112,12 +114,13 @@
     }
 }
 __global__ __launch_bounds__(TB) void k_cas_wpack(const sa_t *__restrict__ src_pos, const u32 *__restrict__ src_val, const u32 *__restrict__ src_rank, u32 rcap,
-                                                  const u32 *__restrict__ region_cnt, const u32 *__restrict__ region_off, sa_t *__restrict__ w_pos, u32 *__restrict__ w_val,
-                                                  u32 *__restrict__ w_rank) {
+                                                  const u32 *__restrict__ region_cnt, sa_t *__restrict__ w_pos, u32 *__restrict__ w_val, u32 *__restrict__ w_rank) {
     const u32 reg = blockIdx.y, i = blockIdx.x * TB + threadIdx.x;
     if (i >= region_cnt[reg]) return;
     const size_t f = (size_t)reg * rcap + i;
-    const u32 o = region_off[reg] + i;
+    u32 off = 0;
+    for (u32 r = 0; r < reg; r++) off += region_cnt[r];
+    const u32 o = off + i;
     w_pos[o] = src_pos[f]; w_val[o] = src_val[f]; w_rank[o] = src_rank[f];
 }
 __global__ __launch_bounds__(TB) void k_cas_wkeys(const u32 *__restrict__ w_rank, u32 NW, u64 *__restrict__ keys, u32 *__restrict__ vals) {
@@ -226,7 +229,9 @@
 __global__ __launch_bounds__(TB) void k_cas_assign(const sa_t *__restrict__ c_pa, const sa_t *__restrict__ c_pb, const u32 *__restrict__ c_len, u32 *__restrict__ c_child,
                                                    u32 M, const sa_t *__restrict__ w_pos, const u32 *__restrict__ w_val, u32 *__restrict__ w_child, u32 NW,
                                                    const CasIv *__restrict__ iv, const CasRes *__restrict__ res, u64 *__restrict__ best, u32 *__restrict__ wmax,
-                                                   int64_t minl, int first, const u64 *__restrict__ ceil ) {
+                                                   int64_t minl, int first, const u64 *__restrict__ ceil ,
+                                                   const u32 *__restrict__ counters ) {
+    if (!first && counters && counters[C_LO] == counters[C_HI]) return;
     const u32 mblocks = (M + TB * CAS_ITEMS - 1) / (TB * CAS_ITEMS);
     for (int it = 0; it < CAS_ITEMS; it++) {
     if (blockIdx.x < mblocks) {
@@ -295,9 +300,10 @@
 
 __global__ __launch_bounds__(TB) void k_cas_winner(const sa_t *__restrict__ c_pa, const sa_t *__restrict__ c_pb, const u32 *__restrict__ c_len,
                                                    const u32 *__restrict__ c_child, u32 M, const CasIv *__restrict__ iv, CasRes *__restrict__ res,
-                                                   const u64 *__restrict__ best, int64_t minl) {
+                                                   const u64 *__restrict__ best, int64_t minl, const u32 *__restrict__ counters) {
     const u32 i = blockIdx.x * TB + threadIdx.x;
     if (i >= M) return;
+    if (counters && counters[C_LO] == counters[C_HI]) return;
     const u32 c = c_child[i];
     if (c == NONE) return;
     int64_t qa, qb, ql;
@@ -489,7 +495,8 @@
 
 __global__ __launch_bounds__(TB) void k_cas_decide(CasIv *__restrict__ iv, u64 *__restrict__ best, u32 *__restrict__ wmax, int32_t *__restrict__ depth,
                                                    CasRes *__restrict__ res, u32 minl, u32 *__restrict__ counters, u32 child_cap,
-                                                   u32 *__restrict__ und_list, u32 leaf_n, RvCascadeIO io, CasDanger dg, int danger) {
+                                                   u32 *__restrict__ und_list, u32 leaf_n, RvCascadeIO io, CasDanger dg, int danger,
+                                                   u32 *__restrict__ landing ) {
     __shared__ u32 s_cnt[TB / 64][3];
     __shared__ u32 s_base[3];
     const u32 lo = counters[C_LO], hi = counters[C_HI];
@@ -591,6 +598,10 @@
             counters[C_LO] = hi; counters[C_HI] = atomicAdd(&counters[C_NCHILD], 0u);
             counters[C_NANCH] = atomicAdd(io.anchor_count, 0u);
             counters[C_TICKET] = 0;
+            if (landing) {
+                for (int k = 0; k < 16; k++) landing[k] = (k == C_TICKET) ? 0u : atomicAdd(&counters[k], 0u);
+                __threadfence_system();
+            }
         }
     }
 }
@@ -881,6 +892,31 @@
     if (bout.cap < 4096 * sizeof(RvPairRec)) RV_TRY(bout.reserve(sizeof(RvPairRec) * (size_t)std::max<int64_t>(4096, n / 64)));
     u32 *tilecnt = btab.as<u32>(), *tileovf = tilecnt + (ntile + 1), *tileoff = tileovf + (ntile + 1);
     u32 M = reuse ? cb.M : 0;
+    const int64_t rcap64 = std::min<int64_t>(n / WT_REGIONS + WT_TILE, std::max<int64_t>(16384, n / 1024));
+    const u32 wcap = (u32)std::min<int64_t>(rcap64 * WT_REGIONS, 0x7fffffff);
+    const u32 wrcap = wcap / WT_REGIONS;
+    DBuf &bwp0 = cb.d[19], &bwv0 = cb.d[20], &bwr = cb.d[21], &bwrk = cb.d[22], &bwrk0 = cb.d[23];
+    RV_TRY(bwp0.reserve((size_t)wcap * sizeof(sa_t))); RV_TRY(bwv0.reserve((size_t)wcap * 4)); RV_TRY(bwr.reserve(2 * WT_REGIONS * 4 + 64));
+    RV_TRY(bwrk.reserve((size_t)wcap * 4)); RV_TRY(bwrk0.reserve((size_t)wcap * 4));
+    u32 *const wreg = bwr.as<u32>();
+    hipStream_t side = (host && host->side && host->side != q) ? host->side : nullptr;
+    struct WitFence {
+        hipStream_t q; hipEvent_t ev = nullptr; bool started = false, pending = false;
+        void wait() { if (pending) { (void)hipStreamWaitEvent(q, ev, 0); pending = false; } }
+        ~WitFence() { wait(); }
+    } wit{q};
+    auto witness_pass = [&](hipStream_t s) -> int {
+        RV_HIP(hipMemsetAsync(wreg, 0, 2 * WT_REGIONS * 4, s));
+        hipLaunchKernelGGL(k_cas_witness, dim3((unsigned)ceil_div(n, WT_TILE)), dim3(TB), 0, s, SA, LCP, BWT, n, minl, bwp0.as<sa_t>(), bwv0.as<u32>(), bwrk0.as<u32>(), wrcap, wreg);
+        RV_LAUNCH_CHECK();
+        return 0;
+    };
+    for (int k = 0; k < 4; k++) cb.tail[k] = 0;
+    if (side) {
+        for (hipEvent_t *e : {&cb.ev_scan, &cb.ev_wit, &cb.ev_land[0], &cb.ev_land[1]}) if (!*e) RV_HIP(hipEventCreateWithFlags(e, hipEventDisableTiming));
+    } else {
+        for (hipEvent_t *e : {&cb.ev_land[0], &cb.ev_land[1]}) if (!*e) RV_HIP(hipEventCreateWithFlags(e, hipEventDisableTiming));
+    }
     for (int attempt = 0; !reuse; attempt++) {
         if (attempt == 3) { rv_set_error("cascade: scan buffer sizing failed"); return -1; }
         const size_t ocap = bout.cap / sizeof(RvPairRec) - RV_PAIR_HDR, vcap = bovf.cap / sizeof(RvPairRec);
@@ -888,6 +924,14 @@
         (void)h->prof.attach(RV_K_SCAN_PAIR, (double)n * 8.0, &ev_a, &ev_b);
         RV_TRY(rv_scan_pair_launch(ws, SA, LCP, n, BWT, (sa_t)h->nsep[0], (int)minl, bslot.as<RvPairRec>(), bovf.as<RvPairRec>(),
                                    (u32)std::min<size_t>(vcap, 0xffffffffu), bcnt.as<u32>(), tilecnt, tileovf, nullptr, nullptr, 0, ev_a, ev_b));
+        if (side && !wit.started) {
+            RV_HIP(hipEventRecord(cb.ev_scan, q));
+            RV_HIP(hipStreamWaitEvent(side, cb.ev_scan, 0));
+            RV_TRY(witness_pass(side));
+            RV_HIP(hipEventRecord(cb.ev_wit, side));
+            wit.ev = cb.ev_wit; wit.started = wit.pending = true;
+            cb.tail[3] = 1;
+        }
         RV_TRY(rv_exclusive_sum_u32(ws, tilecnt, tileoff, ntile + 1));
         RV_TRY(rv_pair_compact_launch(ws, bslot.as<RvPairRec>(), bovf.as<RvPairRec>(), tilecnt, tileovf, tileoff, ntile, bout.as<RvPairRec>(),
                                       (u32)std::min<size_t>(ocap, 0xffffffffu), bcnt.as<u32>(), nullptr, (u32)std::min<size_t>(vcap, 0xffffffffu)));
@@ -905,8 +949,6 @@
     const RvPairRec *recs = bout.as<RvPairRec>() + RV_PAIR_HDR;
     cb.M = M;
 
-    const int64_t rcap64 = std::min<int64_t>(n / WT_REGIONS + WT_TILE, std::max<int64_t>(16384, n / 1024));
-    const u32 wcap = (u32)std::min<int64_t>(rcap64 * WT_REGIONS, 0x7fffffff);
     const int64_t ccap64 = n / (int64_t)minl + 16;
     if (ccap64 >= 0x7fffffff) GIVE_UP("too many sub-indices possible");
     const u32 ccap = (u32)ccap64;
@@ -920,17 +962,10 @@
     u32 *counters = bctr.as<u32>();
     RV_HIP(hipMemsetAsync(counters, 0, 64, q));
 
-    DBuf &bwp0 = cb.d[19], &bwv0 = cb.d[20], &bwr = cb.d[21], &bwrk = cb.d[22], &bwrk0 = cb.d[23];
-    RV_TRY(bwp0.reserve((size_t)wcap * sizeof(sa_t))); RV_TRY(bwv0.reserve((size_t)wcap * 4)); RV_TRY(bwr.reserve(2 * WT_REGIONS * 4 + 64));
-    RV_TRY(bwrk.reserve((size_t)wcap * 4)); RV_TRY(bwrk0.reserve((size_t)wcap * 4));
     u32 hc[16];
     u32 NW = reuse ? cb.NW : 0;
     if (!reuse) {
-        u32 *wreg = bwr.as<u32>();
-        RV_HIP(hipMemsetAsync(wreg, 0, 2 * WT_REGIONS * 4, q));
-        const u32 wrcap = wcap / WT_REGIONS;
-        hipLaunchKernelGGL(k_cas_witness, dim3((unsigned)ceil_div(n, WT_TILE)), dim3(TB), 0, q, SA, LCP, BWT, n, minl, bwp0.as<sa_t>(), bwv0.as<u32>(), bwrk0.as<u32>(), wrcap, wreg);
-        RV_LAUNCH_CHECK();
+        if (!wit.started) RV_TRY(witness_pass(q));
         {
             const unsigned mb = (unsigned)ceil_div((int64_t)M, TB);
             hipLaunchKernelGGL(k_cas_keys, dim3(mb), dim3(TB), 0, q, recs, M, k0.as<u64>(), v0.as<u32>());
@@ -941,17 +976,16 @@
                                blen.as<u32>(), bcc.as<u32>());
             RV_LAUNCH_CHECK();
         }
-        u32 hreg[2 * WT_REGIONS];
+        wit.wait();
+        u32 hreg[WT_REGIONS];
         RV_TRY(rv_read_back(ws, hreg, wreg, WT_REGIONS * 4));
         u32 wmaxc = 0;
-        for (int r = 0; r < WT_REGIONS; r++) { hreg[WT_REGIONS + r] = NW; NW += hreg[r]; wmaxc = std::max(wmaxc, hreg[r]); }
+        for (int r = 0; r < WT_REGIONS; r++) { NW += hreg[r]; wmaxc = std::max(wmaxc, hreg[r]); }
         out->witnesses = NW;
         if (wmaxc > wrcap) GIVE_UP("too many repeat witnesses (a repetitive input)");
         if (NW) {
-            RV_HIP(hipMemcpyAsync(wreg + WT_REGIONS, hreg + WT_REGIONS, WT_REGIONS * 4, hipMemcpyHostToDevice, q));
-            RV_HIP(hipStreamSynchronize(q));
             hipLaunchKernelGGL(k_cas_wpack, dim3((unsigned)std::max<int64_t>(1, ceil_div((int64_t)wmaxc, TB)), WT_REGIONS), dim3(TB), 0, q, (const sa_t *)bwp0.as<sa_t>(),
-                               (const u32 *)bwv0.as<u32>(), (const u32 *)bwrk0.as<u32>(), wrcap, (const u32 *)wreg, (const u32 *)(wreg + WT_REGIONS), bwp.as<sa_t>(), bwv.as<u32>(),
+                               (const u32 *)bwv0.as<u32>(), (const u32 *)bwrk0.as<u32>(), wrcap, (const u32 *)wreg, bwp.as<sa_t>(), bwv.as<u32>(),
                                bwrk.as<u32>());
             RV_LAUNCH_CHECK();
         }
@@ -1045,7 +1079,7 @@
 
     if (verbose) { (void)hipStreamSynchronize(q); tp[2] = cas_now(); }
     const unsigned agrid = (unsigned)(ceil_div((int64_t)M, TB * CAS_ITEMS) + ceil_div((int64_t)NW, TB * CAS_ITEMS));
-    const int batch = std::max(1, (int)ws.opt.cascade_batch);
+    const int batch = ws.opt.cascade_batch > 0 ? (int)ws.opt.cascade_batch : 4;
     int queued = 0;
     RV_TRY(rv_working_text_begin(h, host ? host->side : nullptr));
     u32 sent = 0, known = 0;
@@ -1056,6 +1090,32 @@
         sent = known;
         return 0;
     };
+    u32 filled = 0;
+    struct OffsetFiller {
+        int64_t *off = nullptr; int64_t base = 0;
+        std::atomic<u32> target{0}; std::atomic<bool> stop{false};
+        std::thread th;
+        void start(int64_t *o, int64_t b) {
+            off = o; base = b;
+            th = std::thread([this]() {
+                u32 done = 0;
+                for (int idle = 0;;) {
+                    const u32 t = target.load(std::memory_order_acquire);
+                    if (done < t) { for (u32 k = done; k < t; k++) off[k] = base + 2 * ((int64_t)k + 1); done = t; idle = 0; continue; }
+                    if (stop.load(std::memory_order_acquire)) return;
+                    if (++idle < 256) __builtin_ia32_pause(); else std::this_thread::yield();
+                }
+            });
+        }
+        void finish() { if (th.joinable()) { stop.store(true, std::memory_order_release); th.join(); } }
+        ~OffsetFiller() { finish(); }
+    } filler;
+    auto fill_known = [&]() {
+        if (!host || !host->side || !host->l || !host->off || known <= filled || known > host->cap) return;
+        if (!filler.th.joinable()) filler.start(host->off, host->off_base);
+        filler.target.store(known, std::memory_order_release);
+        filled = known; cb.tail[1] = filled;
+    };
     struct PrioScope {
         Workspace &w; hipStream_t home; RvCascadeBufs &cb; bool on = false;
         ~PrioScope() { leave(); }
@@ -1080,14 +1140,17 @@
         ws.stream = cb.prio_stream; prio.on = true;
         q = cb.prio_stream;
     }
-    for (;;) {
+    RV_TRY(cb.hland.reserve(2 * 64));
+    u32 *const land[2] = {cb.hland.as<u32>(), cb.hland.as<u32>() + 16};
+    const u32 *const empty_ok = (danger && NW) ? nullptr : (const u32 *)counters;
+    auto queue_batch = [&](int slot) -> int {
         for (int b = 0; b < batch; b++, queued++) {
             hipLaunchKernelGGL(k_cas_assign, dim3(agrid), dim3(TB), 0, q, (const sa_t *)bpa.as<sa_t>(), (const sa_t *)bpb.as<sa_t>(), (const u32 *)blen.as<u32>(), bcc.as<u32>(), M,
                                wp, wv, bwc.as<u32>(), NW, (const CasIv *)biv.as<CasIv>(), (const CasRes *)bres.as<CasRes>(),
-                               bbest.as<u64>(), bwm.as<u32>(), (int64_t)minl, queued == 0 ? 1 : 0, (const u64 *)((danger && NW) ? dg.ceil : nullptr));
+                               bbest.as<u64>(), bwm.as<u32>(), (int64_t)minl, queued == 0 ? 1 : 0, (const u64 *)((danger && NW) ? dg.ceil : nullptr), empty_ok);
             RV_LAUNCH_CHECK();
             hipLaunchKernelGGL(k_cas_winner, dim3((unsigned)ceil_div((int64_t)M, TB)), dim3(TB), 0, q, (const sa_t *)bpa.as<sa_t>(), (const sa_t *)bpb.as<sa_t>(),
-                               (const u32 *)blen.as<u32>(), (const u32 *)bcc.as<u32>(), M, (const CasIv *)biv.as<CasIv>(), bres.as<CasRes>(), (const u64 *)bbest.as<u64>(), (int64_t)minl);
+                               (const u32 *)blen.as<u32>(), (const u32 *)bcc.as<u32>(), M, (const CasIv *)biv.as<CasIv>(), bres.as<CasRes>(), (const u64 *)bbest.as<u64>(), (int64_t)minl, empty_ok);
             RV_LAUNCH_CHECK();
             if (danger && NW) {
                 const unsigned wb = (unsigned)ceil_div((int64_t)NW, TB);
@@ -1108,15 +1171,27 @@
                 RV_LAUNCH_CHECK();
             }
             hipLaunchKernelGGL(k_cas_decide, dim3(256), dim3(TB), 0, q, biv.as<CasIv>(), bbest.as<u64>(), bwm.as<u32>(), bdep.as<int32_t>(),
-                               bres.as<CasRes>(), minl, counters, ccap, bund.as<u32>(), (u32)RV_LEAF_N, io, dg, (danger && NW) ? 1 : 0);
+                               bres.as<CasRes>(), minl, counters, ccap, bund.as<u32>(), (u32)RV_LEAF_N, io, dg, (danger && NW) ? 1 : 0, b + 1 == batch ? land[slot] : nullptr);
             RV_LAUNCH_CHECK();
         }
-        RV_TRY(send_known());
-        RV_TRY(rv_read_back(ws, hc, counters, sizeof hc));
+        RV_HIP(hipEventRecord(cb.ev_land[slot], q));
+        return 0;
+    };
+    RV_TRY(queue_batch(0));
+    for (int cur = 0;; cur++) {
+        RV_TRY(queue_batch((cur + 1) & 1));
+        cb.tail[2]++;
+        {
+            const hipError_t e = rv_event_wait(cb.ev_land[cur & 1]);
+            if (e != hipSuccess) { rv_set_error("cascade: %s", hipGetErrorString(e)); return -1; }
+            memcpy(hc, land[cur & 1], sizeof hc);
+        }
         if (hc[C_ERR] & ~5u) { rv_set_error("cascade: device error %u", hc[C_ERR]); return -1; }
         if (hc[C_ERR]) GIVE_UP("the cascade's tables are full");
         known = hc[C_NANCH];
         if (hc[C_MAXN] > (u32)RV_LEAF_N) break;
+        RV_TRY(send_known());
+        fill_known();
         if (hc[C_HI] == hc[C_LO]) break;
         if (queued > 1000000) { rv_set_error("cascade: no progress"); return -1; }
     }
@@ -1134,7 +1209,6 @@
     }
     hipLaunchKernelGGL(k_cas_stats, dim3(256), dim3(TB), 0, q, (const u32 *)counters, (const int32_t *)bdep.as<int32_t>(), io);
     RV_LAUNCH_CHECK();
-    RV_TRY(send_known());
     if (chain) {
         hipLaunchKernelGGL(k_cas_lineage_stats, dim3(1), dim3(64), 0, q, io.stats, (unsigned long long)cb.lin_steps, (unsigned long long)cb.lin_maxdepth);
         RV_LAUNCH_CHECK();
@@ -1178,8 +1252,9 @@
         fprintf(stderr, "cascade%s: %u matches, %u witnesses, %d levels, %u sub-indices, %u undecided (%lld ranks rebuilt), %lld decided from witnesses | ms: scan %.2f witnesses+sort %.2f levels %.2f rebuild+leaf %.2f\n",
                 danger ? " (second attempt)" : "", M, NW, level, hi, U, (long long)out->rebuilt_ranks, (long long)out->solved, (tp[1] - tp[0]) * 1e3, (tp[2] - tp[1]) * 1e3, (tp[3] - tp[2]) * 1e3, (tp[4] - tp[3]) * 1e3);
     }
+    filler.finish();
     out->done = true;
-    out->sent = sent;
+    out->sent = sent; out->filled = filled;
     return 0;
 #undef GIVE_UP
 }
diff --git a/reveal_amd/csrc/rv_cascade_multi.hip b/reveal_amd/csrc/rv_cascade_multi.hip
--- a/reveal_amd/csrc/rv_cascade_multi.hip
+++ b/reveal_amd/csrc/rv_cascade_multi.hip
@@ -1027,7 +1027,7 @@
     hipLaunchKernelGGL(k_cmj_init, dim3((unsigned)ceil_div((int64_t)J, 64)), dim3(64), 0, q, t, k, (const sa_t *)(dsm + o_rb), (const sa_t *)(dsm + o_re), J, counters);
     RV_LAUNCH_CHECK();
     const unsigned agrid = (unsigned)(ceil_div((int64_t)M, TB) + ceil_div((int64_t)NW, TB));
-    const int batch = std::max(1, (int)ws.opt.cascade_batch);
+    const int batch = ws.opt.cascade_batch > 0 ? (int)ws.opt.cascade_batch : 8;
     const u32 big_min = (u32)std::min<int64_t>(jobs[0]->big_min, 0x7fffffff);
     u32 hc[16];
     int queued = 0;
@@ -1284,7 +1284,7 @@
     hipLaunchKernelGGL(k_casm_init, dim3((unsigned)std::max<int64_t>(1, ceil_div((int64_t)NW, TB))), dim3(TB), 0, q, t, k, d_rb, d_re, counters, bwc.as<u32>(), NW);
     RV_LAUNCH_CHECK();
     const unsigned agrid = (unsigned)(ceil_div((int64_t)M, TB) + ceil_div((int64_t)NW, TB));
-    const int batch = std::max(1, (int)ws.opt.cascade_batch);
+    const int batch = ws.opt.cascade_batch > 0 ? (int)ws.opt.cascade_batch : 8;
     int queued = 0;
     for (;;) {
         for (int b = 0; b < batch; b++, queued++) {
diff --git a/reveal_amd/csrc/rv_common.h b/reveal_amd/csrc/rv_common.h
--- a/reveal_amd/csrc/rv_common.h
+++ b/reveal_amd/csrc/rv_common.h
@@ -63,7 +63,7 @@
     X(pb_refresh_tmin, "RV_PB_REFRESH_TMIN", 0) \
     X(cascade_log, "RV_CASCADE_LOG", 0) \
     X(cascade_danger_min, "RV_CASCADE_DANGER_MIN", 0) \
-    X(cascade_batch, "RV_CASCADE_BATCH", 8) \
+    X(cascade_batch, "RV_CASCADE_BATCH", 0)  \
     X(lcp_by_rank, "RV_LCP_BY_RANK", 0) \
     X(no_tiny_sa, "RV_NO_TINY_SA", 0) \
     X(no_short_alphabet, "RV_NO_SHORT_ALPHABET", 0) \
```

Measured after the change: 23680. Within noise of the previous version (-1.0%).
